# popgenmethods/smcpp

Measured on AMD Instinct MI355X. Metric: E-step loglik-evals/sec (100 Mbp, M=64, n=20), higher is better.
Workload: dtype f64 state + f32 scans (mixed)

## Files before the change

### smcpp_amd/csrc/chains_ss.hpp

```cpp
#pragma once

namespace smcpp_dev {

struct SsArgs {
    int M, Mp, nchunks, pass, K, nlds;
    const Chunk *chunks;
    const Chunk *chunks_b;
    int nchunks_b;
    const int *tasks;
    const int2 *rowdesc;
    const double *E;
    const float *pi_f;
    const double *f_dc, *f_g, *f_cg, *f_b, *f_a, *f_d;
    const double *b_dc, *b_g, *b_b, *b_a;
    double c0;
    float *alpha;
    double *beta, *cnorm;
    float *ends_f, *used_f;
    double *ends_b, *used_b;
    int *changed_f, *changed_b;
    int *endchg_f, *endchg_b;
    float eps_f;
    double eps_b;
    int full_f, full_b;
    int mode_f, mode_b;
    int halo = 0;
    long long *dbg;
    int mixed = 0;
    int dirsplit = 0;
    int hyb_th = 0x7fffffff, Ke = 0, hot_ek = 0;
    int nk_lds = 0, key_of_slot[4] = {0, 1, 2, 3}, slot_of_key[4] = {0, 1, 2, 3};
    const double *Pinvrm = nullptr, *Prm = nullptr, *PinvT = nullptr, *PT = nullptr;
    const double *dsc = nullptr;
};

constexpr int SS_KE_MAX = 4;
constexpr int SS_ROW_CONT = 1 << 30;
template <int NPL>
__device__ __forceinline__ float ss_floor_of(int descx) { return (NPL >= 2 && (descx & SS_ROW_CONT)) ? 0.f : 1e-10f; }
template <int NPL>
__device__ __forceinline__ float ss_floor_at(const SsArgs &a, long long row) { return NPL >= 2 ? ss_floor_of<NPL>(a.rowdesc[row].x) : 1e-10f; }

template <int CTRL>
__device__ __forceinline__ double dpp0(double v) {
    const long long x = __builtin_bit_cast(long long, v);
    int lo = (int)(x & 0xffffffffll), hi = (int)(x >> 32);
    lo = __builtin_amdgcn_update_dpp(0, lo, CTRL, 0xf, 0xf, true);
    hi = __builtin_amdgcn_update_dpp(0, hi, CTRL, 0xf, 0xf, true);
    return __builtin_bit_cast(double, ((long long)hi << 32) | (unsigned int)lo);
}
template <int CTRL>
__device__ __forceinline__ float dpp0(float v) {
    return __builtin_bit_cast(float, __builtin_amdgcn_update_dpp(0, __builtin_bit_cast(int, v), CTRL, 0xf, 0xf, true));
}

constexpr int DPP_SHR1 = 0x111, DPP_SHR2 = 0x112, DPP_SHR4 = 0x114, DPP_SHR8 = 0x118, DPP_BC15 = 0x142, DPP_BC31 = 0x143,
              DPP_WSHR1 = 0x138;

template <typename T>
__device__ __forceinline__ T ss_scan(T v, T c15, T c31) {
    v += dpp0<DPP_SHR1>(v);
    v += dpp0<DPP_SHR2>(v);
    v += dpp0<DPP_SHR4>(v);
    v += dpp0<DPP_SHR8>(v);
    v = __builtin_fma(c15, dpp0<DPP_BC15>(v), v);
    v = __builtin_fma(c31, dpp0<DPP_BC31>(v), v);
    return v;
}
__device__ __forceinline__ float ss_scan_f(float v, float c15, float c31) {
    v += dpp0<DPP_SHR1>(v);
    v += dpp0<DPP_SHR2>(v);
    v += dpp0<DPP_SHR4>(v);
    v += dpp0<DPP_SHR8>(v);
    v = __builtin_fmaf(c15, dpp0<DPP_BC15>(v), v);
    v = __builtin_fmaf(c31, dpp0<DPP_BC31>(v), v);
    return v;
}
__device__ __forceinline__ double ss_scan_w(double v, const double (&lv)[6]) {
    v = __builtin_fma(lv[0], dpp0<DPP_SHR1>(v), v);
    v = __builtin_fma(lv[1], dpp0<DPP_SHR2>(v), v);
    v = __builtin_fma(lv[2], dpp0<DPP_SHR4>(v), v);
    v = __builtin_fma(lv[3], dpp0<DPP_SHR8>(v), v);
    v = __builtin_fma(lv[4], dpp0<DPP_BC15>(v), v);
    v = __builtin_fma(lv[5], dpp0<DPP_BC31>(v), v);
    return v;
}
__device__ __forceinline__ void ss_levels(double A, int lane, double (&lv)[6]) {
    const int r = lane & 15, row = lane >> 4;
    double m = A, t;
    lv[0] = m; t = dpp0<DPP_SHR1>(m); m = (r >= 1) ? m * t : m;
    lv[1] = m; t = dpp0<DPP_SHR2>(m); m = (r >= 2) ? m * t : m;
    lv[2] = m; t = dpp0<DPP_SHR4>(m); m = (r >= 4) ? m * t : m;
    lv[3] = m; t = dpp0<DPP_SHR8>(m); m = (r >= 8) ? m * t : m;
    lv[4] = (row & 1) ? m : 0.0; t = dpp0<DPP_BC15>(m); m = (row & 1) ? m * t : m;
    lv[5] = (row >= 2) ? m : 0.0;
}

template <int NPL>
struct SsFwdC {
    double dc[NPL], g[NPL], cg[NPL], b[NPL], a[NPL], d[NPL], cumA[NPL], lv[6], c15, c31;
    float lvf[6];
    double adg;
    float bgf, bff, c0f, m1, m2, m3;
};
template <int NPL>
struct SsBwdC {
    double dc[NPL], g[NPL], b[NPL], a[NPL], cumA[NPL], lv[6], c15, c31, c0;
    float c15f, c31f, lvf[6];
    double adg;
    float gf, bff, c0f, m1, m2, m3;
};

template <int NPL>
__device__ __forceinline__ void ss_load_fwd(const SsArgs &a, int lane, SsFwdC<NPL> &c) {
    double cum = 1.0;
#pragma unroll
    for (int k = 0; k < NPL; ++k) {
        const int p = lane * NPL + k;
        c.dc[k] = a.f_dc[p]; c.g[k] = a.f_g[p]; c.cg[k] = a.f_cg[p]; c.b[k] = a.f_b[p]; c.a[k] = a.f_a[p]; c.d[k] = a.f_d[p];
        cum *= c.a[k];
        c.cumA[k] = cum;
    }
    ss_levels(cum, lane, c.lv);
#pragma unroll
    for (int q = 0; q < 6; ++q) c.lvf[q] = (float)c.lv[q];
    const int row = lane >> 4;
    c.c15 = (row & 1) ? 1.0 : 0.0;
    c.c31 = (row >= 2) ? 1.0 : 0.0;
    c.adg = c.d[0] - c.g[0];
    c.bgf = (float)(c.g[0] - a.c0); c.bff = (float)c.b[0]; c.c0f = (float)a.c0;
    c.m1 = row < 1 ? 1.f : 0.f; c.m2 = row < 2 ? 1.f : 0.f; c.m3 = row < 3 ? 1.f : 0.f;
}
template <int NPL>
__device__ __forceinline__ void ss_load_bwd(const SsArgs &a, int lane, SsBwdC<NPL> &c) {
    double cum = 1.0;
#pragma unroll
    for (int k = 0; k < NPL; ++k) {
        const int p = lane * NPL + k;
        c.dc[k] = a.b_dc[p]; c.g[k] = a.b_g[p]; c.b[k] = a.b_b[p]; c.a[k] = a.b_a[p];
        cum *= c.a[k];
        c.cumA[k] = cum;
    }
    ss_levels(cum, lane, c.lv);
    const int row = lane >> 4;
    c.c15 = (row & 1) ? 1.0 : 0.0;
    c.c31 = (row >= 2) ? 1.0 : 0.0;
    c.c15f = (float)c.c15; c.c31f = (float)c.c31;
#pragma unroll
    for (int q = 0; q < 6; ++q) c.lvf[q] = (float)c.lv[q];
    c.c0 = a.c0;
    c.adg = c.dc[0] - c.g[0];
    c.gf = (float)c.g[0]; c.bff = (float)c.b[0]; c.c0f = (float)a.c0;
    c.m1 = row < 1 ? 1.f : 0.f; c.m2 = row < 2 ? 1.f : 0.f; c.m3 = row < 3 ? 1.f : 0.f;
}

#define SS_D_ " row_mask:0xf bank_mask:0xf bound_ctrl:1\n"
template <bool H32>
__device__ __forceinline__ void ss_x_scan_fwd(float &z, float &s, float &zp, float &tot, const float (&lv)[6], float m1, float m2,
                                              float m3, float bg, float c0) {
    float t1, t2, t3;
    if (H32) {
        asm volatile("s_nop 1\n"
                     "v_add_f32_dpp %1, %1, %1 row_shl:1" SS_D_ "v_fmac_f32_dpp %0, %0, %5 row_shr:1" SS_D_ "s_nop 0\n"
                     "v_add_f32_dpp %1, %1, %1 row_shl:2" SS_D_ "v_fmac_f32_dpp %0, %0, %6 row_shr:2" SS_D_ "s_nop 0\n"
                     "v_add_f32_dpp %1, %1, %1 row_shl:4" SS_D_ "v_fmac_f32_dpp %0, %0, %7 row_shr:4" SS_D_ "s_nop 0\n"
                     "v_add_f32_dpp %1, %1, %1 row_shl:8" SS_D_ "v_fmac_f32_dpp %0, %0, %8 row_shr:8" SS_D_
                     "v_readlane_b32 %4, %1, 16\n"
                     "s_nop 0\n"
                     "v_fmac_f32_dpp %0, %0, %9 row_bcast:15" SS_D_
                     "v_fmac_f32_e32 %1, %4, %10\n"
                     "s_nop 0\n"
                     "v_readlane_b32 %3, %1, 0\n"
                     "v_mov_b32_dpp %2, %0 wave_shr:1" SS_D_
                     "v_fmac_f32_e32 %2, %11, %1\n"
                     "v_fmac_f32_e32 %2, %3, %12\n"
                     : "+v"(z), "+v"(s), "=&v"(zp), "=&s"(tot), "=&s"(t1)
                     : "v"(lv[0]), "v"(lv[1]), "v"(lv[2]), "v"(lv[3]), "v"(lv[4]), "v"(m1), "v"(bg), "v"(c0));
        return;
    }
    asm volatile("s_nop 1\n"
                 "v_add_f32_dpp %1, %1, %1 row_shl:1" SS_D_ "v_fmac_f32_dpp %0, %0, %7 row_shr:1" SS_D_ "s_nop 0\n"
                 "v_add_f32_dpp %1, %1, %1 row_shl:2" SS_D_ "v_fmac_f32_dpp %0, %0, %8 row_shr:2" SS_D_ "s_nop 0\n"
                 "v_add_f32_dpp %1, %1, %1 row_shl:4" SS_D_ "v_fmac_f32_dpp %0, %0, %9 row_shr:4" SS_D_ "s_nop 0\n"
                 "v_add_f32_dpp %1, %1, %1 row_shl:8" SS_D_ "v_fmac_f32_dpp %0, %0, %10 row_shr:8" SS_D_
                 "v_readlane_b32 %4, %1, 16\n"
                 "v_readlane_b32 %5, %1, 32\n"
                 "v_fmac_f32_dpp %0, %0, %11 row_bcast:15" SS_D_
                 "v_readlane_b32 %6, %1, 48\n"
                 "v_fmac_f32_e32 %1, %4, %13\n"
                 "v_fmac_f32_dpp %0, %0, %12 row_bcast:31" SS_D_
                 "v_fmac_f32_e32 %1, %5, %14\n"
                 "v_fmac_f32_e32 %1, %6, %15\n"
                 "v_mov_b32_dpp %2, %0 wave_shr:1" SS_D_
                 "v_readlane_b32 %3, %1, 0\n"
                 "v_fmac_f32_e32 %2, %16, %1\n"
                 "s_nop 0\n"
                 "v_fmac_f32_e32 %2, %3, %17\n"
                 : "+v"(z), "+v"(s), "=&v"(zp), "=&s"(tot), "=&s"(t1), "=&s"(t2), "=&s"(t3)
                 : "v"(lv[0]), "v"(lv[1]), "v"(lv[2]), "v"(lv[3]), "v"(lv[4]), "v"(lv[5]), "v"(m1), "v"(m2), "v"(m3), "v"(bg), "v"(c0));
}
template <bool H32>
__device__ __forceinline__ void ss_x_scan_bwd(float &v, float &f, float &gs, float &tot, const float (&lv)[6], float c15, float c31,
                                              float m1, float m2, float m3, float b, float c0) {
    float t1, t2, t3, vp;
    if (H32) {
        asm volatile("s_nop 1\n"
                     "v_add_f32_dpp %1, %0, %0 row_shr:1" SS_D_ "v_add_f32_dpp %2, %2, %2 row_shl:1" SS_D_ "v_fmac_f32_dpp %0, %0, %6 row_shr:1" SS_D_
                     "v_add_f32_dpp %1, %1, %1 row_shr:2" SS_D_ "v_add_f32_dpp %2, %2, %2 row_shl:2" SS_D_ "v_fmac_f32_dpp %0, %0, %7 row_shr:2" SS_D_
                     "v_add_f32_dpp %1, %1, %1 row_shr:4" SS_D_ "v_add_f32_dpp %2, %2, %2 row_shl:4" SS_D_ "v_fmac_f32_dpp %0, %0, %8 row_shr:4" SS_D_
                     "v_add_f32_dpp %1, %1, %1 row_shr:8" SS_D_ "v_add_f32_dpp %2, %2, %2 row_shl:8" SS_D_ "v_fmac_f32_dpp %0, %0, %9 row_shr:8" SS_D_
                     "v_readlane_b32 %5, %2, 48\n"
                     "v_fmac_f32_dpp %1, %1, %11 row_bcast:15" SS_D_
                     "v_fmac_f32_dpp %0, %0, %10 row_bcast:15" SS_D_
                     "v_fmac_f32_e32 %2, %5, %12\n"
                     "v_readlane_b32 %3, %1, 63\n"
                     "v_mov_b32_dpp %4, %0 wave_shr:1" SS_D_
                     "v_fmac_f32_e32 %2, %14, %1\n"
                     "v_fmac_f32_e32 %2, %13, %4\n"
                     : "+v"(v), "=&v"(f), "+v"(gs), "=&s"(tot), "=&v"(vp), "=&s"(t3)
                     : "v"(lv[0]), "v"(lv[1]), "v"(lv[2]), "v"(lv[3]), "v"(lv[4]), "v"(c15), "v"(m3), "v"(b), "v"(c0));
        return;
    }
    asm volatile("s_nop 1\n"
                 "v_add_f32_dpp %1, %0, %0 row_shr:1" SS_D_ "v_add_f32_dpp %2, %2, %2 row_shl:1" SS_D_ "v_fmac_f32_dpp %0, %0, %8 row_shr:1" SS_D_
                 "v_add_f32_dpp %1, %1, %1 row_shr:2" SS_D_ "v_add_f32_dpp %2, %2, %2 row_shl:2" SS_D_ "v_fmac_f32_dpp %0, %0, %9 row_shr:2" SS_D_
                 "v_add_f32_dpp %1, %1, %1 row_shr:4" SS_D_ "v_add_f32_dpp %2, %2, %2 row_shl:4" SS_D_ "v_fmac_f32_dpp %0, %0, %10 row_shr:4" SS_D_
                 "v_add_f32_dpp %1, %1, %1 row_shr:8" SS_D_ "v_add_f32_dpp %2, %2, %2 row_shl:8" SS_D_ "v_fmac_f32_dpp %0, %0, %11 row_shr:8" SS_D_
                 "v_readlane_b32 %5, %2, 16\n"
                 "v_fmac_f32_dpp %1, %1, %14 row_bcast:15" SS_D_
                 "v_fmac_f32_dpp %0, %0, %12 row_bcast:15" SS_D_
                 "v_readlane_b32 %6, %2, 32\n"
                 "v_readlane_b32 %7, %2, 48\n"
                 "v_fmac_f32_dpp %1, %1, %15 row_bcast:31" SS_D_
                 "v_fmac_f32_dpp %0, %0, %13 row_bcast:31" SS_D_
                 "v_fmac_f32_e32 %2, %5, %16\n"
                 "v_fmac_f32_e32 %2, %6, %17\n"
                 "v_fmac_f32_e32 %2, %7, %18\n"
                 "v_mov_b32_dpp %4, %0 wave_shr:1" SS_D_
                 "v_readlane_b32 %3, %1, 63\n"
                 "v_fmac_f32_e32 %2, %20, %1\n"
                 "v_fmac_f32_e32 %2, %19, %4\n"
                 : "+v"(v), "=&v"(f), "+v"(gs), "=&s"(tot), "=&v"(vp), "=&s"(t1), "=&s"(t2), "=&s"(t3)
                 : "v"(lv[0]), "v"(lv[1]), "v"(lv[2]), "v"(lv[3]), "v"(lv[4]), "v"(lv[5]), "v"(c15), "v"(c31), "v"(m1), "v"(m2), "v"(m3),
                   "v"(b), "v"(c0));
}
#undef SS_D_

template <int NPL, bool MIX = false, bool H32 = false>
__device__ __forceinline__ void ss_fwd_step(const SsFwdC<NPL> &c, const double (&x)[NPL], const double (&e)[NPL],
                                            double (&out)[NPL], double &S) {
    if (MIX && NPL == 1) {
        float s = (float)x[0];
        float z = c.bff * s, zp, tot;
        ss_x_scan_fwd<H32>(z, s, zp, tot, c.lvf, c.m1, c.m2, c.m3, c.bgf, c.c0f);
        S = (double)tot;
        out[0] = e[0] * __builtin_fma(c.adg, x[0], (double)zp);
        return;
    }
    double lp[NPL], w[NPL];
    lp[0] = x[0];
    w[0] = c.b[0] * x[0];
#pragma unroll
    for (int k = 1; k < NPL; ++k) {
        lp[k] = lp[k - 1] + x[k];
        w[k] = __builtin_fma(c.a[k], w[k - 1], c.b[k] * x[k]);
    }
    double p_ = lp[NPL - 1], z_ = w[NPL - 1];
    {
        double tp, tz;
        tp = dpp0<DPP_SHR1>(p_); tz = dpp0<DPP_SHR1>(z_); p_ += tp; z_ = __builtin_fma(c.lv[0], tz, z_);
        tp = dpp0<DPP_SHR2>(p_); tz = dpp0<DPP_SHR2>(z_); p_ += tp; z_ = __builtin_fma(c.lv[1], tz, z_);
        tp = dpp0<DPP_SHR4>(p_); tz = dpp0<DPP_SHR4>(z_); p_ += tp; z_ = __builtin_fma(c.lv[2], tz, z_);
        tp = dpp0<DPP_SHR8>(p_); tz = dpp0<DPP_SHR8>(z_); p_ += tp; z_ = __builtin_fma(c.lv[3], tz, z_);
        tp = dpp0<DPP_BC15>(p_); tz = dpp0<DPP_BC15>(z_); p_ = __builtin_fma(c.c15, tp, p_); z_ = __builtin_fma(c.lv[4], tz, z_);
        tp = dpp0<DPP_BC31>(p_); tz = dpp0<DPP_BC31>(z_); p_ = __builtin_fma(c.c31, tp, p_); z_ = __builtin_fma(c.lv[5], tz, z_);
    }
    const double li = p_, LI = z_;
    S = lane_get(li, 63);
    const double LIp = dpp0<DPP_WSHR1>(LI);
    if (NPL == 1) {
        out[0] = e[0] * __builtin_fma(c.dc[0], x[0], __builtin_fma(c.g[0], S, __builtin_fma(c.cg[0], li, LIp)));
        return;
    }
    const double lex = li - lp[NPL - 1];
#pragma unroll
    for (int k = 0; k < NPL; ++k) {
        const double incl = lex + lp[k];
        const double Z = (k == 0) ? LIp : __builtin_fma(c.cumA[k - 1 < 0 ? 0 : k - 1], LIp, w[k - 1 < 0 ? 0 : k - 1]);
        const double t = __builtin_fma(c.dc[k], x[k], __builtin_fma(c.g[k], S, __builtin_fma(c.cg[k], incl, Z)));
        out[k] = e[k] * t;
    }
}

template <int NPL, bool MIX = false, bool H32 = false>
__device__ __forceinline__ void ss_bwd_step(const SsBwdC<NPL> &c, const double (&bv)[NPL], const double (&e)[NPL],
                                            double (&out)[NPL], float &Sw) {
    if (MIX && NPL == 1) {
        const double w0 = e[0] * bv[0];
        float v = (float)w0;
        float gs = c.gf * v, f;
        ss_x_scan_bwd<H32>(v, f, gs, Sw, c.lvf, c.c15f, c.c31f, c.m1, c.m2, c.m3, c.bff, c.c0f);
        out[0] = __builtin_fma(c.adg, w0, (double)gs);
        return;
    }
    double w[NPL], lg[NPL], u[NPL];
    float lf[NPL];
#pragma unroll
    for (int k = 0; k < NPL; ++k) w[k] = e[k] * bv[k];
    lg[0] = c.g[0] * w[0];
    u[0] = w[0];
    lf[0] = (float)w[0];
#pragma unroll
    for (int k = 1; k < NPL; ++k) {
        lg[k] = __builtin_fma(c.g[k], w[k], lg[k - 1]);
        u[k] = __builtin_fma(c.a[k], u[k - 1], w[k]);
        lf[k] = lf[k - 1] + (float)w[k];
    }
    double p_ = lg[NPL - 1], z_ = u[NPL - 1];
    float f_ = lf[NPL - 1];
    {
        double tp, tz;
        float tf;
        tp = dpp0<DPP_SHR1>(p_); tz = dpp0<DPP_SHR1>(z_); tf = dpp0<DPP_SHR1>(f_); p_ += tp; z_ = __builtin_fma(c.lv[0], tz, z_); f_ += tf;
        tp = dpp0<DPP_SHR2>(p_); tz = dpp0<DPP_SHR2>(z_); tf = dpp0<DPP_SHR2>(f_); p_ += tp; z_ = __builtin_fma(c.lv[1], tz, z_); f_ += tf;
        tp = dpp0<DPP_SHR4>(p_); tz = dpp0<DPP_SHR4>(z_); tf = dpp0<DPP_SHR4>(f_); p_ += tp; z_ = __builtin_fma(c.lv[2], tz, z_); f_ += tf;
        tp = dpp0<DPP_SHR8>(p_); tz = dpp0<DPP_SHR8>(z_); tf = dpp0<DPP_SHR8>(f_); p_ += tp; z_ = __builtin_fma(c.lv[3], tz, z_); f_ += tf;
        tp = dpp0<DPP_BC15>(p_); tz = dpp0<DPP_BC15>(z_); tf = dpp0<DPP_BC15>(f_);
        p_ = __builtin_fma(c.c15, tp, p_); z_ = __builtin_fma(c.lv[4], tz, z_); f_ = __builtin_fmaf(c.c15f, tf, f_);
        tp = dpp0<DPP_BC31>(p_); tz = dpp0<DPP_BC31>(z_); tf = dpp0<DPP_BC31>(f_);
        p_ = __builtin_fma(c.c31, tp, p_); z_ = __builtin_fma(c.lv[5], tz, z_); f_ = __builtin_fmaf(c.c31f, tf, f_);
    }
    const double lig = p_, LI = z_;
    const float lif = f_;
    const double Gtot = lane_get(lig, 63);
    Sw = lane_get(lif, 63);
    const double LIp = dpp0<DPP_WSHR1>(LI);
    if (NPL == 1) {
        out[0] = __builtin_fma(c.dc[0], w[0], (Gtot - lig) + __builtin_fma(c.c0, (double)lif, c.b[0] * LIp));
        return;
    }
    const double lexg = lig - lg[NPL - 1];
    const float lexf = lif - lf[NPL - 1];
#pragma unroll
    for (int k = 0; k < NPL; ++k) {
        const double inclG = lexg + lg[k];
        const double inclW = (double)(lexf + lf[k]);
        const double V = (k == 0) ? LIp : __builtin_fma(c.cumA[k - 1 < 0 ? 0 : k - 1], LIp, u[k - 1 < 0 ? 0 : k - 1]);
        out[k] = __builtin_fma(c.dc[k], w[k], (Gtot - inclG) + __builtin_fma(c.c0, inclW, c.b[k] * V));
    }
}

__device__ __forceinline__ void ss_desc_settle(int2 &d) { asm volatile("" : "+v"(d.x), "+v"(d.y)); }
__device__ __forceinline__ void ss_vm_drain() { __builtin_amdgcn_s_waitcnt(0x0F70); }
__device__ __forceinline__ int ss_uni(int v) { return __builtin_amdgcn_readfirstlane(v); }
__device__ __forceinline__ Chunk ss_uniform_chunk(const Chunk &c) {
    Chunk u;
    const unsigned lo = (unsigned)__builtin_amdgcn_readfirstlane((int)(c.base & 0xffffffffll));
    const unsigned hi = (unsigned)__builtin_amdgcn_readfirstlane((int)(c.base >> 32));
    u.base = (long long)(((unsigned long long)hi << 32) | lo);
    u.r0 = ss_uni(c.r0); u.r1 = ss_uni(c.r1); u.contig = ss_uni(c.contig); u.first = ss_uni(c.first); u.last = ss_uni(c.last);
    u.pad = ss_uni(c.pad); u.h0 = ss_uni(c.h0); u.h1 = ss_uni(c.h1);
    return u;
}

template <int NPL, bool BWD, bool ALLLDS = false>
__device__ __forceinline__ void ss_emission(const SsArgs &a, const double *sE, int slot, int lane, double (&e)[NPL]) {
    constexpr int MS = 64 * NPL;
    if (ALLLDS || slot < a.nlds) {
        const double *src = sE + (size_t)slot * MS;
#pragma unroll
        for (int k = 0; k < NPL; ++k) e[k] = src[BWD ? MS - 1 - (lane * NPL + k) : lane * NPL + k];
    } else {
        const double *src = a.E + (size_t)slot * MS;
#pragma unroll
        for (int k = 0; k < NPL; ++k) e[k] = src[BWD ? MS - 1 - (lane * NPL + k) : lane * NPL + k];
    }
}

__device__ __forceinline__ double ss_sum_halves(double v) {
    const long long x = __builtin_bit_cast(long long, v);
    const int lo = (int)(x & 0xffffffffll), hi = (int)(x >> 32);
    const auto r0 = __builtin_amdgcn_permlane32_swap(lo, lo, false, false);
    const auto r1 = __builtin_amdgcn_permlane32_swap(hi, hi, false, false);
    const double a = __builtin_bit_cast(double, ((long long)(unsigned)r1[0] << 32) | (unsigned)r0[0]);
    const double b = __builtin_bit_cast(double, ((long long)(unsigned)r1[1] << 32) | (unsigned)r0[1]);
    return a + b;
}
__device__ __forceinline__ double ss_exp_neg(double x) {
    if (!(x > -745.0)) return 0.0;
    const double n = __builtin_rint(x * 1.4426950408889634);
    double r = __builtin_fma(-n, 6.93147180369123816490e-01, x);
    r = __builtin_fma(-n, 1.90821492927058770002e-10, r);
    double p = 1.0 / 6227020800.0;
    p = __builtin_fma(p, r, 1.0 / 479001600.0);
    p = __builtin_fma(p, r, 1.0 / 39916800.0);
    p = __builtin_fma(p, r, 1.0 / 3628800.0);
    p = __builtin_fma(p, r, 1.0 / 362880.0);
    p = __builtin_fma(p, r, 1.0 / 40320.0);
    p = __builtin_fma(p, r, 1.0 / 5040.0);
    p = __builtin_fma(p, r, 1.0 / 720.0);
    p = __builtin_fma(p, r, 1.0 / 120.0);
    p = __builtin_fma(p, r, 1.0 / 24.0);
    p = __builtin_fma(p, r, 1.0 / 6.0);
    p = __builtin_fma(p, r, 0.5);
    p = __builtin_fma(p, r, 1.0);
    p = __builtin_fma(p, r, 1.0);
    return ldexp(p, (int)n);
}
struct SsEigC { double ld[SS_KE_MAX]; bool neg[SS_KE_MAX]; int slot[SS_KE_MAX]; int r, g, nb, G, tpk; };
__device__ __forceinline__ void ss_load_eig(const SsArgs &a, int lp, SsEigC &c) {
    c.G = a.Mp <= 32 ? 2 : 1;
    c.tpk = a.dirsplit ? 2 : 4;
    const int W = 64 / c.G;
    c.r = lp & (W - 1); c.g = lp / W; c.nb = a.Mp / c.G;
#pragma unroll
    for (int e = 0; e < SS_KE_MAX; ++e) {
        double d = 0.0;
        if (e < a.Ke && c.r < a.M) d = a.dsc[(size_t)e * a.Mp + c.r];
        c.ld[e] = log(fabs(d));
        c.neg[e] = d < 0.0;
        c.slot[e] = a.slot_of_key[e];
    }
}
__device__ __forceinline__ double ss_eig_pow(const SsEigC &c, int ek, int span) {
    double l = c.ld[0];
    bool ng = c.neg[0];
#pragma unroll
    for (int e = 1; e < SS_KE_MAX; ++e) if (ek == e) { l = c.ld[e]; ng = c.neg[e]; }
    const double p = ss_exp_neg((double)span * l);
    return (ng && (span & 1)) ? -p : p;
}
__device__ __forceinline__ double ss_eig_matvec(const SsEigC &c, const double *tab, int Mp, int slot, int which, double *sx, int lp, double x) {
    sx[lp] = x;
    wave_lds_fence();
    const double *row = tab + ((size_t)(slot * c.tpk + (which & (c.tpk - 1))) * Mp + min(c.r, Mp - 1)) * (Mp + 1) + c.g * c.nb;
    const double *xv = sx + c.g * c.nb;
    double a0 = 0.0, a1 = 0.0;
    for (int b = 0; b < c.nb; b += 4) {
        const double r0 = row[b], r1 = row[b + 1], r2 = row[b + 2], r3 = row[b + 3];
        const double v0 = xv[b], v1 = xv[b + 1], v2 = xv[b + 2], v3 = xv[b + 3];
        a0 = __builtin_fma(r0, v0, a0); a1 = __builtin_fma(r1, v1, a1);
        a0 = __builtin_fma(r2, v2, a0); a1 = __builtin_fma(r3, v3, a1);
    }
    double acc = a0 + a1;
    if (c.G >= 2) acc = ss_sum_halves(acc);
    wave_lds_fence();
    return acc;
}
__device__ __forceinline__ double ss_eig_matvec_cold(const SsEigC &c, const double *mat, int Mp, double *sx, int lp, double x) {
    sx[lp] = x;
    wave_lds_fence();
    const double *row = mat + (size_t)min(c.r, Mp - 1) * Mp + c.g * c.nb;
    const double *xv = sx + c.g * c.nb;
    double a0 = 0.0, a1 = 0.0;
    for (int b = 0; b < c.nb; b += 8) {
        double rr[8];
#pragma unroll
        for (int q = 0; q < 8; ++q) rr[q] = row[b + q];
#pragma unroll
        for (int q = 0; q < 8; q += 2) { a0 = __builtin_fma(rr[q], xv[b + q], a0); a1 = __builtin_fma(rr[q + 1], xv[b + q + 1], a1); }
    }
    double acc = a0 + a1;
    if (c.G >= 2) acc = ss_sum_halves(acc);
    wave_lds_fence();
    return acc;
}

template <int NB>
struct SsHotRows { double a[NB], b[NB]; };
template <int NB>
__device__ __forceinline__ void ss_eig_rows(const SsEigC &c, const double *tab, int Mp, int ek, int w0, double (&ra)[NB], double (&rb)[NB]) {
    const size_t rowoff = (size_t)min(c.r, Mp - 1) * (Mp + 1) + c.g * NB;
    const double *rowA = tab + (size_t)(ek * c.tpk + (w0 & (c.tpk - 1))) * Mp * (Mp + 1) + rowoff;
    const double *rowB = tab + (size_t)(ek * c.tpk + (w0 & (c.tpk - 1)) + 1) * Mp * (Mp + 1) + rowoff;
#pragma unroll
    for (int b = 0; b < NB; ++b) { ra[b] = rowA[b]; rb[b] = rowB[b]; }
}
template <int NB>
__device__ __forceinline__ double ss_eig_step(const SsEigC &c, const double *tab, int Mp, int ek, int w0, double *sx, int lp,
                                              double xin, int span, const SsHotRows<NB> &hot, int hot_ek) {
    double ra[NB], rb[NB];
    if (ek == hot_ek) {
#pragma unroll
        for (int b = 0; b < NB; ++b) { ra[b] = hot.a[b]; rb[b] = hot.b[b]; }
    } else ss_eig_rows<NB>(c, tab, Mp, ek, w0, ra, rb);
    sx[lp] = xin;
    const double pw = ss_eig_pow(c, ek, span);
    wave_lds_fence();
    const double *xv = sx + c.g * NB;
    double a0 = 0.0, a1 = 0.0;
#pragma unroll
    for (int b = 0; b < NB; b += 2) { a0 = __builtin_fma(ra[b], xv[b], a0); a1 = __builtin_fma(ra[b + 1], xv[b + 1], a1); }
    const double u = ss_sum_halves(a0 + a1) * pw;
    wave_lds_fence();
    sx[c.r] = u;
    wave_lds_fence();
    a0 = 0.0; a1 = 0.0;
#pragma unroll
    for (int b = 0; b < NB; b += 2) { a0 = __builtin_fma(rb[b], xv[b], a0); a1 = __builtin_fma(rb[b + 1], xv[b + 1], a1); }
    const double o = ss_sum_halves(a0 + a1);
    wave_lds_fence();
    return o;
}
__device__ __forceinline__ double ss_eig_apply(const SsArgs &a, const SsEigC &c, const double *tab, int Mp, int ek, int w0, double *sx, int lp,
                                               double xin, int span, const SsHotRows<16> &hot, int hot_ek) {
    if (Mp == 32) return ss_eig_step<16>(c, tab, Mp, ek, w0, sx, lp, xin, span, hot, hot_ek);
    if (Mp == 16) {
        SsHotRows<8> none;
        return ss_eig_step<8>(c, tab, Mp, ek, w0, sx, lp, xin, span, none, -1);
    }
    int slot = c.slot[0];
#pragma unroll
    for (int e = 1; e < SS_KE_MAX; ++e) if (ek == e) slot = c.slot[e];
    if (slot >= 0) {
        double u = ss_eig_matvec(c, tab, Mp, slot, w0, sx, lp, xin);
        u *= ss_eig_pow(c, ek, span);
        return ss_eig_matvec(c, tab, Mp, slot, w0 + 1, sx, lp, lp < 64 / c.G ? u : 0.0);
    }
    const size_t MM = (size_t)Mp * Mp;
    const double *m0 = (w0 == 0 ? a.Pinvrm : a.PT) + (size_t)ek * MM, *m1 = (w0 == 0 ? a.Prm : a.PinvT) + (size_t)ek * MM;
    double u = ss_eig_matvec_cold(c, m0, Mp, sx, lp, xin);
    u *= ss_eig_pow(c, ek, span);
    return ss_eig_matvec_cold(c, m1, Mp, sx, lp, lp < 64 / c.G ? u : 0.0);
}

template <int NPL, bool ALLLDS>
__device__ __forceinline__ void ss_fwd_light_rows(const SsArgs &a, const double *sE, long long base, int first, int last, int lane, float (&x)[NPL]);
template <int NPL, bool ALLLDS>
__device__ __forceinline__ void ss_bwd_light_rows(const SsArgs &a, const double *sE, long long base, int rhi, int rlo, int lane, float (&b)[NPL]);

template <int NPL, bool RERUN, bool HYB, bool ALLLDS, bool MIX = false, bool H32 = false>
__device__ __forceinline__ void ss_forward_wave(const SsArgs &a, const double *sE, int c, int lane) {
    constexpr int MS = 64 * NPL;
    const int M = a.M, Mp = a.Mp, pass = a.pass;
    const Chunk ch = ss_uniform_chunk(a.chunks[c]);
    float *end_cur = a.ends_f + ((size_t)(pass & 1) * a.nchunks + c) * Mp;
    const float *end_prev = a.ends_f + ((size_t)((pass + 1) & 1) * a.nchunks + c) * Mp;
    int st[NPL];
    bool live[NPL], stor[NPL];
#pragma unroll
    for (int k = 0; k < NPL; ++k) { st[k] = lane * NPL + k; live[k] = st[k] < M; stor[k] = st[k] < Mp; }
    if (RERUN && ch.first && !a.full_f) {
#pragma unroll
        for (int k = 0; k < NPL; ++k) if (stor[k]) end_cur[st[k]] = end_prev[st[k]];
        return;
    }
    double x[NPL];
    {
        const float *src = (ch.first || !RERUN) ? a.pi_f : a.ends_f + ((size_t)((pass + 1) & 1) * a.nchunks + (c - 1)) * Mp;
#pragma unroll
        for (int k = 0; k < NPL; ++k) x[k] = live[k] ? (double)src[st[k]] : 0.0;
    }
    const bool halo = !RERUN && !HYB && a.halo && ch.h0 < ch.r0;
    const int rbeg = halo ? ch.h1 : ch.r0;
    const int jst = ch.r0 - rbeg;
    if (halo && ch.h0 < ch.h1) {
        float xf[NPL];
#pragma unroll
        for (int k = 0; k < NPL; ++k) xf[k] = (float)x[k];
        ss_fwd_light_rows<NPL, ALLLDS>(a, sE, ch.base, ch.h0, ch.h1, lane, xf);
#pragma unroll
        for (int k = 0; k < NPL; ++k) x[k] = live[k] ? (double)xf[k] : 0.0;
        if (jst == 0) {
            double part = 0.0;
#pragma unroll
            for (int k = 0; k < NPL; ++k) part += x[k];
            const double iv = 1.0 / wave_sum_dpp(part);
#pragma unroll
            for (int k = 0; k < NPL; ++k) {
                const float an = live[k] ? fmaxf((float)(x[k] * iv), ss_floor_at<NPL>(a, ch.base + ch.r0 + 1)) : 0.f;
                x[k] = (double)an;
                if (stor[k]) a.used_f[(size_t)c * Mp + st[k]] = an;
            }
        }
    }
    if (RERUN && !a.full_f) {
        bool diff = false;
#pragma unroll
        for (int k = 0; k < NPL; ++k)
            if (live[k]) {
                const float u = a.used_f[(size_t)c * Mp + st[k]];
                if (!(fabsf((float)x[k] - u) <= a.eps_f * fabsf(u))) diff = true;
            }
        if (!__any(diff)) {
#pragma unroll
            for (int k = 0; k < NPL; ++k) if (stor[k]) end_cur[st[k]] = end_prev[st[k]];
            return;
        }
    }
    if (!halo) {
#pragma unroll
        for (int k = 0; k < NPL; ++k) if (stor[k]) a.used_f[(size_t)c * Mp + st[k]] = (float)x[k];
    }
    if (lane == 0) a.changed_f[pass] = 1;
    if (ch.first) {
#pragma unroll
        for (int k = 0; k < NPL; ++k) if (stor[k]) a.alpha[(size_t)ch.base * Mp + st[k]] = (float)x[k];
        if (lane == 0) a.cnorm[ch.base] = 1.0;
    }
    SsFwdC<NPL> cst;
    ss_load_fwd<NPL>(a, lane, cst);
    const int2 *rd = a.rowdesc + ch.base + rbeg + 1;
    const int nrows = ch.r1 - rbeg;
    int2 dcur = rd[lane], dnxt = rd[64 + lane];
    ss_desc_settle(dcur); ss_desc_settle(dnxt);
    float *arow = a.alpha + (size_t)(ch.base + rbeg) * Mp;
    double *crow = a.cnorm + ch.base + rbeg;
    float *ap[NPL];
#pragma unroll
    for (int k = 0; k < NPL; ++k) ap[k] = arow + st[k];
    int cacc = 0;
    auto cflush = [&](int jhi) {
        const int jj = (jhi & ~63) + lane;
        if (jj <= jhi && jj > jst && jj > 0) crow[jj] = (double)__builtin_bit_cast(float, cacc);
    };
    double e[NPL];
    ss_emission<NPL, false, ALLLDS>(a, sE, __builtin_amdgcn_readlane(dcur.x, 0) & 0xFFFF, lane, e);
    constexpr bool hyb = HYB && NPL == 1;
    const double *tab = sE + (size_t)a.nlds * MS;
    SsEigC ec;
    SsHotRows<16> hot;
    int hot_ek = -1;
    if (hyb) {
        ss_load_eig(a, lane, ec);
        if (Mp == 32) { hot_ek = a.hot_ek; ss_eig_rows<16>(ec, tab, Mp, hot_ek, 0, hot.a, hot.b); }
    }
    double *sxw = const_cast<double *>(tab) + (size_t)a.nk_lds * (a.dirsplit ? 2 : 4) * Mp * (Mp + 1) + (threadIdx.x >> 6) * 64;
    bool merged = false;
    const long long t0c = __builtin_readcyclecounter(), t0r = __builtin_amdgcn_s_memrealtime();
    long long npos = 0;
    ss_vm_drain();
    for (int j = 0; j < nrows; ++j) {
        const int jl = j & 63;
        const int span = __builtin_amdgcn_readlane(dcur.y, jl);
        const int ekr = (__builtin_amdgcn_readlane(dcur.x, jl) >> 16) & 0xFF;
        const float flo = NPL >= 2 ? ss_floor_of<NPL>(__builtin_amdgcn_readlane(dcur.x, jl)) : 1e-10f;
        npos += span;
        if (jl == 63) { dcur = dnxt; dnxt = rd[j + 65 + lane]; ss_desc_settle(dnxt); }
        if (MIX && jl == 0 && j > 0) cflush(j - 1);
        const int slot_n = __builtin_amdgcn_readlane(dcur.x, (j + 1) & 63) & 0xFFFF;
        double en[NPL];
        ss_emission<NPL, false, ALLLDS>(a, sE, slot_n, lane, en);
        if (hyb && span > a.hyb_th) {
            const double S = wave_sum_dpp(x[0]);
            const double inv = rcp_f64(S);
            double xin = x[0] * inv;
            if (j > 0) {
                const float an = live[0] ? fmaxf((float)xin, flo) : 0.f;
                if (RERUN && !a.full_f && (j & 15) == 0 && j >= 16) {
                    bool bad = false;
                    if (live[0]) {
                        const float old = arow[(size_t)j * Mp + st[0]];
                        if (!(fabsf(an - old) <= a.eps_f * fabsf(old))) bad = true;
                    }
                    if (!__any(bad)) { merged = true; break; }
                }
                if (stor[0]) arow[(size_t)j * Mp + st[0]] = an;
                if (lane == 0) crow[j] = S;
                xin = (double)an;
            }
            const double xo = ss_eig_apply(a, ec, tab, Mp, ekr, 0, sxw, lane, xin, span, hot, hot_ek);
            x[0] = live[0] ? xo : 0.0;
#pragma unroll
            for (int k = 0; k < NPL; ++k) e[k] = en[k];
            continue;
        }
        double y[NPL], S;
        ss_fwd_step<NPL, MIX, MIX && H32>(cst, x, e, y, S);
        double inv;
        if (MIX) {
            const double r0 = (double)__builtin_amdgcn_rcpf((float)S);
            inv = __builtin_fma(__builtin_fma(-S, r0, 1.0), r0, r0);
        } else inv = rcp_f64(S);
        double fb[NPL];
#pragma unroll
        for (int k = 0; k < NPL; ++k) fb[k] = 0.0;
        if (j > 0) {
            float an[NPL];
#pragma unroll
            for (int k = 0; k < NPL; ++k) {
                const double xs = x[k] * inv;
                an[k] = live[k] ? fmaxf((float)xs, flo) : 0.f;
                fb[k] = (double)an[k] - xs;
            }
            if (RERUN && !a.full_f && (j & 15) == 0 && j >= 16) {
                bool bad = false;
#pragma unroll
                for (int k = 0; k < NPL; ++k)
                    if (live[k]) {
                        const float old = MIX ? *ap[k] : arow[(size_t)j * Mp + st[k]];
                        if (!(fabsf(an[k] - old) <= a.eps_f * fabsf(old))) bad = true;
                    }
                if (!__any(bad)) { merged = true; if (MIX) cflush(j - 1); break; }
            }
            if (j > jst) {
                if (MIX) {
#pragma unroll
                    for (int k = 0; k < NPL; ++k) if (stor[k]) *ap[k] = an[k];
                    cacc = lane == jl ? __builtin_bit_cast(int, (float)S) : cacc;
                } else {
#pragma unroll
                    for (int k = 0; k < NPL; ++k) if (stor[k]) arow[(size_t)j * Mp + st[k]] = an[k];
                    if (lane == 0) crow[j] = S;
                }
            } else if (j == jst) {
#pragma unroll
                for (int k = 0; k < NPL; ++k) if (stor[k]) a.used_f[(size_t)c * Mp + st[k]] = an[k];
            }
        }
#pragma unroll
        for (int k = 0; k < NPL; ++k) {
            double ed = e[k] * cst.d[k];
            if (span == 1) { const double edf = (double)(float)ed; y[k] = __builtin_fma(edf - ed, x[k], y[k]); ed = edf; }
            x[k] = __builtin_fma(ed, fb[k], y[k] * inv);
        }
        {
            double S2;
            int t = 1;
            for (; t + 1 < span; t += 2) {
                ss_fwd_step<NPL, MIX, MIX && H32>(cst, x, e, y, S2);
#pragma unroll
                for (int k = 0; k < NPL; ++k) x[k] = y[k];
                ss_fwd_step<NPL, MIX, MIX && H32>(cst, x, e, y, S2);
#pragma unroll
                for (int k = 0; k < NPL; ++k) x[k] = y[k];
            }
            if (t < span) {
                ss_fwd_step<NPL, MIX, MIX && H32>(cst, x, e, y, S2);
#pragma unroll
                for (int k = 0; k < NPL; ++k) x[k] = y[k];
            }
        }
#pragma unroll
        for (int k = 0; k < NPL; ++k) e[k] = en[k];
        if (MIX) {
#pragma unroll
            for (int k = 0; k < NPL; ++k) ap[k] += Mp;
        }
    }
    if (MIX && !merged && nrows > 0) cflush(nrows - 1);
    if (a.dbg && !RERUN && c == 1 && lane == 0) {
        a.dbg[0] = __builtin_readcyclecounter() - t0c; a.dbg[1] = __builtin_amdgcn_s_memrealtime() - t0r;
        a.dbg[2] = npos; a.dbg[3] = nrows;
    }
    if (merged) {
#pragma unroll
        for (int k = 0; k < NPL; ++k) if (stor[k]) end_cur[st[k]] = end_prev[st[k]];
        return;
    }
    {
        double part = 0.0;
#pragma unroll
        for (int k = 0; k < NPL; ++k) part += x[k];
        const double S = wave_sum_dpp(part);
        const double inv = 1.0 / S;
#pragma unroll
        for (int k = 0; k < NPL; ++k) {
            const float an = live[k] ? fmaxf((float)(x[k] * inv), ss_floor_at<NPL>(a, ch.base + ch.r1 + 1)) : 0.f;
            if (stor[k]) { a.alpha[(size_t)(ch.base + ch.r1) * Mp + st[k]] = an; end_cur[st[k]] = an; }
        }
        if (lane == 0) { a.cnorm[ch.base + ch.r1] = S; a.endchg_f[pass] = 1; }
    }
}

template <int NPL, bool RERUN, bool HYB, bool ALLLDS, bool MIX = false, bool H32 = false>
__device__ __forceinline__ void ss_backward_wave(const SsArgs &a, const double *sE, int c, int lane) {
    constexpr int MS = 64 * NPL;
    const int M = a.M, Mp = a.Mp, pass = a.pass;
    const Chunk ch = ss_uniform_chunk(a.chunks_b[c]);
    double *end_cur = a.ends_b + ((size_t)(pass & 1) * a.nchunks_b + c) * Mp;
    const double *end_prev = a.ends_b + ((size_t)((pass + 1) & 1) * a.nchunks_b + c) * Mp;
    int st[NPL];
    bool live[NPL], stor[NPL];
#pragma unroll
    for (int k = 0; k < NPL; ++k) { st[k] = MS - 1 - (lane * NPL + k); live[k] = st[k] < M; stor[k] = st[k] < Mp; }
    if (RERUN && ch.last && !a.full_b) {
#pragma unroll
        for (int k = 0; k < NPL; ++k) if (stor[k]) end_cur[st[k]] = end_prev[st[k]];
        return;
    }
    double b[NPL];
    {
        const bool fresh = ch.last || !RERUN;
        const double *src = a.ends_b + ((size_t)((pass + 1) & 1) * a.nchunks_b + (fresh ? c : c + 1)) * Mp;
#pragma unroll
        for (int k = 0; k < NPL; ++k) b[k] = live[k] ? (fresh ? 1.0 / (double)M : src[st[k]]) : 0.0;
    }
    const bool halo = !RERUN && !HYB && a.halo && ch.h0 > ch.r1;
    const int rend = halo ? ch.h1 : ch.r1;
    const int jst = rend - ch.r1;
    if (halo && ch.h0 > ch.h1) {
        float bf_[NPL];
#pragma unroll
        for (int k = 0; k < NPL; ++k) bf_[k] = (float)b[k];
        ss_bwd_light_rows<NPL, ALLLDS>(a, sE, ch.base, ch.h0, ch.h1, lane, bf_);
        float pt = 0.f;
#pragma unroll
        for (int k = 0; k < NPL; ++k) pt += live[k] ? bf_[k] : 0.f;
        const float iv = 1.f / wave_sum_dpp(pt);
#pragma unroll
        for (int k = 0; k < NPL; ++k) b[k] = live[k] ? (double)(bf_[k] * iv) : 0.0;
    }
    if (RERUN && !a.full_b) {
        bool diff = false;
#pragma unroll
        for (int k = 0; k < NPL; ++k)
            if (live[k]) {
                const double u = a.used_b[(size_t)c * Mp + st[k]];
                if (!(fabs(b[k] - u) <= a.eps_b * fabs(u))) diff = true;
            }
        if (!__any(diff)) {
#pragma unroll
            for (int k = 0; k < NPL; ++k) if (stor[k]) end_cur[st[k]] = end_prev[st[k]];
            return;
        }
    }
    if (!halo) {
#pragma unroll
        for (int k = 0; k < NPL; ++k) if (stor[k]) a.used_b[(size_t)c * Mp + st[k]] = b[k];
    }
    if (lane == 0) a.changed_b[pass] = 1;
    SsBwdC<NPL> cst;
    ss_load_bwd<NPL>(a, lane, cst);
    const int2 *rd = a.rowdesc + ch.base + rend;
    const int nrows = rend - ch.r0;
    int2 dcur = rd[-lane], dnxt = rd[-64 - lane];
    ss_desc_settle(dcur); ss_desc_settle(dnxt);
    double *brow = a.beta + (size_t)(ch.base + rend) * Mp;
    double *bp[NPL];
#pragma unroll
    for (int k = 0; k < NPL; ++k) bp[k] = brow + st[k];
    double e[NPL];
    ss_emission<NPL, true, ALLLDS>(a, sE, __builtin_amdgcn_readlane(dcur.x, 0) & 0xFFFF, lane, e);
    constexpr bool hyb = HYB && NPL == 1;
    const double *tab = sE + (size_t)a.nlds * MS;
    SsEigC ec;
    SsHotRows<16> hot;
    int hot_ek = -1;
    if (hyb) {
        ss_load_eig(a, 63 - lane, ec);
        if (Mp == 32) { hot_ek = a.hot_ek; ss_eig_rows<16>(ec, tab, Mp, hot_ek, 2, hot.a, hot.b); }
    }
    double *sxw = const_cast<double *>(tab) + (size_t)a.nk_lds * (a.dirsplit ? 2 : 4) * Mp * (Mp + 1) + (threadIdx.x >> 6) * 64;
    bool merged = false;
    const long long t0c = __builtin_readcyclecounter(), t0r = __builtin_amdgcn_s_memrealtime();
    long long npos = 0;
    ss_vm_drain();
    for (int j = 0; j < nrows; ++j) {
        const int jl = j & 63;
        const int span = __builtin_amdgcn_readlane(dcur.y, jl);
        const int ekr = (__builtin_amdgcn_readlane(dcur.x, jl) >> 16) & 0xFF;
        npos += span;
        if (jl == 63) { dcur = dnxt; dnxt = rd[-(j + 65) - lane]; ss_desc_settle(dnxt); }
        const int slot_n = __builtin_amdgcn_readlane(dcur.x, (j + 1) & 63) & 0xFFFF;
        double en[NPL];
        ss_emission<NPL, true, ALLLDS>(a, sE, slot_n, lane, en);
        if (RERUN && !a.full_b && (j & 15) == 0 && j >= 16) {
            bool bad = false;
#pragma unroll
            for (int k = 0; k < NPL; ++k)
                if (live[k]) {
                    const double old = MIX ? *bp[k] : brow[-(ptrdiff_t)j * Mp + st[k]];
                    if (!(fabs(b[k] - old) <= a.eps_b * fabs(old))) bad = true;
                }
            if (!__any(bad)) { merged = true; break; }
        }
        if (halo && j == jst) {
            double part = 0.0;
#pragma unroll
            for (int k = 0; k < NPL; ++k) part += live[k] ? b[k] : 0.0;
            const double iv = 1.0 / wave_sum_dpp(part);
#pragma unroll
            for (int k = 0; k < NPL; ++k) {
                b[k] = live[k] ? b[k] * iv : 0.0;
                if (stor[k]) a.used_b[(size_t)c * Mp + st[k]] = b[k];
            }
        }
        if (j >= jst) {
#pragma unroll
            for (int k = 0; k < NPL; ++k) if (stor[k]) { if (MIX) *bp[k] = b[k]; else brow[-(ptrdiff_t)j * Mp + st[k]] = b[k]; }
        }
        if (hyb && span > a.hyb_th) {
            const double bin = live[0] ? b[0] : 0.0;
            double bo = ss_eig_apply(a, ec, tab, Mp, ekr, 2, sxw, 63 - lane, bin, span, hot, hot_ek);
            bo = live[0] ? bo : 0.0;
            b[0] = bo * rcp_f64(wave_sum_dpp(bo));
#pragma unroll
            for (int k = 0; k < NPL; ++k) e[k] = en[k];
            continue;
        }
        double y[NPL];
        float Sw;
        ss_bwd_step<NPL, MIX, MIX && H32>(cst, b, e, y, Sw);
        const double inv = (double)__builtin_amdgcn_rcpf(Sw);
#pragma unroll
        for (int k = 0; k < NPL; ++k) b[k] = y[k] * inv;
        {
            float S2;
            int t = 1;
            for (; t + 1 < span; t += 2) {
                ss_bwd_step<NPL, MIX, MIX && H32>(cst, b, e, y, S2);
#pragma unroll
                for (int k = 0; k < NPL; ++k) b[k] = y[k];
                ss_bwd_step<NPL, MIX, MIX && H32>(cst, b, e, y, S2);
#pragma unroll
                for (int k = 0; k < NPL; ++k) b[k] = y[k];
            }
            if (t < span) {
                ss_bwd_step<NPL, MIX, MIX && H32>(cst, b, e, y, S2);
#pragma unroll
                for (int k = 0; k < NPL; ++k) b[k] = y[k];
            }
        }
#pragma unroll
        for (int k = 0; k < NPL; ++k) e[k] = en[k];
        if (MIX) {
#pragma unroll
            for (int k = 0; k < NPL; ++k) bp[k] -= Mp;
        }
    }
    if (a.dbg && !RERUN && c == 1 && lane == 0) {
        a.dbg[4] = __builtin_readcyclecounter() - t0c; a.dbg[5] = __builtin_amdgcn_s_memrealtime() - t0r;
        a.dbg[6] = npos; a.dbg[7] = nrows;
    }
    if (merged) {
#pragma unroll
        for (int k = 0; k < NPL; ++k) if (stor[k]) end_cur[st[k]] = end_prev[st[k]];
        return;
    }
    {
        double part = 0.0;
#pragma unroll
        for (int k = 0; k < NPL; ++k) part += live[k] ? b[k] : 0.0;
        const double S = wave_sum_dpp(part);
#pragma unroll
        for (int k = 0; k < NPL; ++k) {
            const double bf = live[k] ? b[k] / S : 0.0;
            if (stor[k]) { end_cur[st[k]] = bf; if (ch.first) a.beta[(size_t)ch.base * Mp + st[k]] = bf; }
        }
        if (lane == 0) a.endchg_b[pass] = 1;
    }
}

template <int NPL>
struct SsLightC { float dc[NPL], g[NPL], cg[NPL], b[NPL], a[NPL], cumA[NPL], lv[6], c15, c31, c0; };

template <int NPL, bool BWD>
__device__ __forceinline__ void ss_load_light(const SsArgs &a, int lane, SsLightC<NPL> &c) {
    double cum = 1.0;
#pragma unroll
    for (int k = 0; k < NPL; ++k) {
        const int p = lane * NPL + k;
        c.dc[k] = (float)(BWD ? a.b_dc[p] : a.f_dc[p]);
        c.g[k] = (float)(BWD ? a.b_g[p] : a.f_g[p]);
        c.cg[k] = BWD ? 0.f : (float)a.f_cg[p];
        c.b[k] = (float)(BWD ? a.b_b[p] : a.f_b[p]);
        const double av = BWD ? a.b_a[p] : a.f_a[p];
        c.a[k] = (float)av;
        cum *= av;
        c.cumA[k] = (float)cum;
    }
    double lv[6];
    ss_levels(cum, lane, lv);
#pragma unroll
    for (int q = 0; q < 6; ++q) c.lv[q] = (float)lv[q];
    const int row = lane >> 4;
    c.c15 = (row & 1) ? 1.f : 0.f;
    c.c31 = (row >= 2) ? 1.f : 0.f;
    c.c0 = (float)a.c0;
}

#define SS_DPP_ "row_mask:0xf bank_mask:0xf bound_ctrl:1\n"
template <bool H32>
__device__ __forceinline__ void ss_light_scan2(float &p, float &z, const float (&lv)[6], float c15, float c31) {
    if (H32) {
        asm volatile("s_nop 1\n"
                     "v_add_f32_dpp %0, %0, %0 row_shr:1 " SS_DPP_ "v_fmac_f32_dpp %1, %1, %2 row_shr:1 " SS_DPP_ "s_nop 0\n"
                     "v_add_f32_dpp %0, %0, %0 row_shr:2 " SS_DPP_ "v_fmac_f32_dpp %1, %1, %3 row_shr:2 " SS_DPP_ "s_nop 0\n"
                     "v_add_f32_dpp %0, %0, %0 row_shr:4 " SS_DPP_ "v_fmac_f32_dpp %1, %1, %4 row_shr:4 " SS_DPP_ "s_nop 0\n"
                     "v_add_f32_dpp %0, %0, %0 row_shr:8 " SS_DPP_ "v_fmac_f32_dpp %1, %1, %5 row_shr:8 " SS_DPP_ "s_nop 0\n"
                     "v_fmac_f32_dpp %0, %0, %7 row_bcast:15 " SS_DPP_ "v_fmac_f32_dpp %1, %1, %6 row_bcast:15 " SS_DPP_ "s_nop 1\n"
                     : "+v"(p), "+v"(z)
                     : "v"(lv[0]), "v"(lv[1]), "v"(lv[2]), "v"(lv[3]), "v"(lv[4]), "v"(c15));
        return;
    }
    asm volatile("s_nop 1\n"
                 "v_add_f32_dpp %0, %0, %0 row_shr:1 " SS_DPP_ "v_fmac_f32_dpp %1, %1, %2 row_shr:1 " SS_DPP_ "s_nop 0\n"
                 "v_add_f32_dpp %0, %0, %0 row_shr:2 " SS_DPP_ "v_fmac_f32_dpp %1, %1, %3 row_shr:2 " SS_DPP_ "s_nop 0\n"
                 "v_add_f32_dpp %0, %0, %0 row_shr:4 " SS_DPP_ "v_fmac_f32_dpp %1, %1, %4 row_shr:4 " SS_DPP_ "s_nop 0\n"
                 "v_add_f32_dpp %0, %0, %0 row_shr:8 " SS_DPP_ "v_fmac_f32_dpp %1, %1, %5 row_shr:8 " SS_DPP_ "s_nop 0\n"
                 "v_fmac_f32_dpp %0, %0, %8 row_bcast:15 " SS_DPP_ "v_fmac_f32_dpp %1, %1, %6 row_bcast:15 " SS_DPP_ "s_nop 0\n"
                 "v_fmac_f32_dpp %0, %0, %9 row_bcast:31 " SS_DPP_ "v_fmac_f32_dpp %1, %1, %7 row_bcast:31 " SS_DPP_ "s_nop 1\n"
                 : "+v"(p), "+v"(z)
                 : "v"(lv[0]), "v"(lv[1]), "v"(lv[2]), "v"(lv[3]), "v"(lv[4]), "v"(lv[5]), "v"(c15), "v"(c31));
}
template <bool H32>
__device__ __forceinline__ void ss_light_scan3(float &p, float &z, float &f, const float (&lv)[6], float c15, float c31) {
    if (H32) {
        asm volatile("s_nop 1\n"
                     "v_add_f32_dpp %0, %0, %0 row_shr:1 " SS_DPP_ "v_fmac_f32_dpp %1, %1, %3 row_shr:1 " SS_DPP_ "v_add_f32_dpp %2, %2, %2 row_shr:1 " SS_DPP_
                     "v_add_f32_dpp %0, %0, %0 row_shr:2 " SS_DPP_ "v_fmac_f32_dpp %1, %1, %4 row_shr:2 " SS_DPP_ "v_add_f32_dpp %2, %2, %2 row_shr:2 " SS_DPP_
                     "v_add_f32_dpp %0, %0, %0 row_shr:4 " SS_DPP_ "v_fmac_f32_dpp %1, %1, %5 row_shr:4 " SS_DPP_ "v_add_f32_dpp %2, %2, %2 row_shr:4 " SS_DPP_
                     "v_add_f32_dpp %0, %0, %0 row_shr:8 " SS_DPP_ "v_fmac_f32_dpp %1, %1, %6 row_shr:8 " SS_DPP_ "v_add_f32_dpp %2, %2, %2 row_shr:8 " SS_DPP_
                     "v_fmac_f32_dpp %0, %0, %8 row_bcast:15 " SS_DPP_ "v_fmac_f32_dpp %1, %1, %7 row_bcast:15 " SS_DPP_ "v_fmac_f32_dpp %2, %2, %8 row_bcast:15 " SS_DPP_ "s_nop 1\n"
                     : "+v"(p), "+v"(z), "+v"(f)
                     : "v"(lv[0]), "v"(lv[1]), "v"(lv[2]), "v"(lv[3]), "v"(lv[4]), "v"(c15));
        return;
    }
    asm volatile("s_nop 1\n"
                 "v_add_f32_dpp %0, %0, %0 row_shr:1 " SS_DPP_ "v_fmac_f32_dpp %1, %1, %3 row_shr:1 " SS_DPP_ "v_add_f32_dpp %2, %2, %2 row_shr:1 " SS_DPP_
                 "v_add_f32_dpp %0, %0, %0 row_shr:2 " SS_DPP_ "v_fmac_f32_dpp %1, %1, %4 row_shr:2 " SS_DPP_ "v_add_f32_dpp %2, %2, %2 row_shr:2 " SS_DPP_
                 "v_add_f32_dpp %0, %0, %0 row_shr:4 " SS_DPP_ "v_fmac_f32_dpp %1, %1, %5 row_shr:4 " SS_DPP_ "v_add_f32_dpp %2, %2, %2 row_shr:4 " SS_DPP_
                 "v_add_f32_dpp %0, %0, %0 row_shr:8 " SS_DPP_ "v_fmac_f32_dpp %1, %1, %6 row_shr:8 " SS_DPP_ "v_add_f32_dpp %2, %2, %2 row_shr:8 " SS_DPP_
                 "v_fmac_f32_dpp %0, %0, %9 row_bcast:15 " SS_DPP_ "v_fmac_f32_dpp %1, %1, %7 row_bcast:15 " SS_DPP_ "v_fmac_f32_dpp %2, %2, %9 row_bcast:15 " SS_DPP_
                 "v_fmac_f32_dpp %0, %0, %10 row_bcast:31 " SS_DPP_ "v_fmac_f32_dpp %1, %1, %8 row_bcast:31 " SS_DPP_ "v_fmac_f32_dpp %2, %2, %10 row_bcast:31 " SS_DPP_ "s_nop 1\n"
                 : "+v"(p), "+v"(z), "+v"(f)
                 : "v"(lv[0]), "v"(lv[1]), "v"(lv[2]), "v"(lv[3]), "v"(lv[4]), "v"(lv[5]), "v"(c15), "v"(c31));
}
#undef SS_DPP_

template <int NPL, bool H32 = false>
__device__ __forceinline__ void ss_fwd_step_f(const SsLightC<NPL> &c, const float (&x)[NPL], const float (&e)[NPL],
                                              float (&out)[NPL], float &S) {
    float lp[NPL], w[NPL];
    lp[0] = x[0];
    w[0] = c.b[0] * x[0];
#pragma unroll
    for (int k = 1; k < NPL; ++k) {
        lp[k] = lp[k - 1] + x[k];
        w[k] = __builtin_fmaf(c.a[k], w[k - 1], c.b[k] * x[k]);
    }
    float p_ = lp[NPL - 1], z_ = w[NPL - 1];
    ss_light_scan2<H32>(p_, z_, c.lv, c.c15, c.c31);
    S = lane_get(p_, H32 ? 31 : 63);
    const float LIp = dpp0<DPP_WSHR1>(z_);
    if (NPL == 1) {
        out[0] = e[0] * __builtin_fmaf(c.dc[0], x[0], __builtin_fmaf(c.g[0], S, __builtin_fmaf(c.cg[0], p_, LIp)));
        return;
    }
    const float lex = p_ - lp[NPL - 1];
#pragma unroll
    for (int k = 0; k < NPL; ++k) {
        const float incl = lex + lp[k];
        const float Z = (k == 0) ? LIp : __builtin_fmaf(c.cumA[k - 1 < 0 ? 0 : k - 1], LIp, w[k - 1 < 0 ? 0 : k - 1]);
        out[k] = e[k] * __builtin_fmaf(c.dc[k], x[k], __builtin_fmaf(c.g[k], S, __builtin_fmaf(c.cg[k], incl, Z)));
    }
}

template <int NPL, bool H32 = false>
__device__ __forceinline__ void ss_bwd_step_f(const SsLightC<NPL> &c, const float (&bv)[NPL], const float (&e)[NPL],
                                              float (&out)[NPL], float &Sw) {
    float w[NPL], lg[NPL], u[NPL], lf[NPL];
#pragma unroll
    for (int k = 0; k < NPL; ++k) w[k] = e[k] * bv[k];
    lg[0] = c.g[0] * w[0];
    u[0] = w[0];
    lf[0] = w[0];
#pragma unroll
    for (int k = 1; k < NPL; ++k) {
        lg[k] = __builtin_fmaf(c.g[k], w[k], lg[k - 1]);
        u[k] = __builtin_fmaf(c.a[k], u[k - 1], w[k]);
        lf[k] = lf[k - 1] + w[k];
    }
    float p_ = lg[NPL - 1], z_ = u[NPL - 1], f_ = lf[NPL - 1];
    ss_light_scan3<H32>(p_, z_, f_, c.lv, c.c15, c.c31);
    const float Gtot = lane_get(p_, 63);
    Sw = lane_get(f_, 63);
    const float LIp = dpp0<DPP_WSHR1>(z_);
    if (NPL == 1) {
        out[0] = __builtin_fmaf(c.dc[0], w[0], (Gtot - p_) + __builtin_fmaf(c.c0, f_, c.b[0] * LIp));
        return;
    }
    const float lexg = p_ - lg[NPL - 1], lexf = f_ - lf[NPL - 1];
#pragma unroll
    for (int k = 0; k < NPL; ++k) {
        const float inclG = lexg + lg[k], inclW = lexf + lf[k];
        const float V = (k == 0) ? LIp : __builtin_fmaf(c.cumA[k - 1 < 0 ? 0 : k - 1], LIp, u[k - 1 < 0 ? 0 : k - 1]);
        out[k] = __builtin_fmaf(c.dc[k], w[k], (Gtot - inclG) + __builtin_fmaf(c.c0, inclW, c.b[k] * V));
    }
}

template <int NPL, bool BWD, bool ALLLDS>
__device__ __forceinline__ void ss_emission_f(const SsArgs &a, const double *sE, int slot, int lane, float (&e)[NPL]) {
    double ed[NPL];
    ss_emission<NPL, BWD, ALLLDS>(a, sE, slot, lane, ed);
#pragma unroll
    for (int k = 0; k < NPL; ++k) e[k] = (float)ed[k];
}

template <int NPL, bool ALLLDS>
__device__ __forceinline__ void ss_fwd_light_rows(const SsArgs &a, const double *sE, long long base, int first, int last, int lane,
                                                  float (&x)[NPL]) {
    SsLightC<NPL> cst;
    ss_load_light<NPL, false>(a, lane, cst);
    const int2 *rd = a.rowdesc + base + first + 1;
    const int nrows = last - first;
    int2 dcur = rd[lane], dnxt = rd[64 + lane];
    ss_desc_settle(dcur); ss_desc_settle(dnxt);
    float e[NPL];
    ss_emission_f<NPL, false, ALLLDS>(a, sE, __builtin_amdgcn_readlane(dcur.x, 0) & 0xFFFF, lane, e);
    ss_vm_drain();
    for (int j = 0; j < nrows; ++j) {
        const int jl = j & 63;
        const int span = __builtin_amdgcn_readlane(dcur.y, jl);
        if (jl == 63) { dcur = dnxt; dnxt = rd[j + 65 + lane]; ss_desc_settle(dnxt); }
        const int slot_n = __builtin_amdgcn_readlane(dcur.x, (j + 1) & 63) & 0xFFFF;
        float en[NPL], y[NPL], S;
        ss_emission_f<NPL, false, ALLLDS>(a, sE, slot_n, lane, en);
        ss_fwd_step_f<NPL>(cst, x, e, y, S);
        const float inv = __builtin_amdgcn_rcpf(S);
#pragma unroll
        for (int k = 0; k < NPL; ++k) x[k] = y[k] * inv;
        float S2;
        int t = 1;
        for (; t + 1 < span; t += 2) {
            ss_fwd_step_f<NPL>(cst, x, e, y, S2);
#pragma unroll
            for (int k = 0; k < NPL; ++k) x[k] = y[k];
            ss_fwd_step_f<NPL>(cst, x, e, y, S2);
#pragma unroll
            for (int k = 0; k < NPL; ++k) x[k] = y[k];
        }
        if (t < span) {
            ss_fwd_step_f<NPL>(cst, x, e, y, S2);
#pragma unroll
            for (int k = 0; k < NPL; ++k) x[k] = y[k];
        }
#pragma unroll
        for (int k = 0; k < NPL; ++k) e[k] = en[k];
    }
}
template <int NPL, bool ALLLDS>
__device__ __forceinline__ void ss_bwd_light_rows(const SsArgs &a, const double *sE, long long base, int rhi, int rlo, int lane,
                                                  float (&b)[NPL]) {
    SsLightC<NPL> cst;
    ss_load_light<NPL, true>(a, lane, cst);
    const int2 *rd = a.rowdesc + base + rhi;
    const int nrows = rhi - rlo;
    int2 dcur = rd[-lane], dnxt = rd[-64 - lane];
    ss_desc_settle(dcur); ss_desc_settle(dnxt);
    float e[NPL];
    ss_emission_f<NPL, true, ALLLDS>(a, sE, __builtin_amdgcn_readlane(dcur.x, 0) & 0xFFFF, lane, e);
    ss_vm_drain();
    for (int j = 0; j < nrows; ++j) {
        const int jl = j & 63;
        const int span = __builtin_amdgcn_readlane(dcur.y, jl);
        if (jl == 63) { dcur = dnxt; dnxt = rd[-(j + 65) - lane]; ss_desc_settle(dnxt); }
        const int slot_n = __builtin_amdgcn_readlane(dcur.x, (j + 1) & 63) & 0xFFFF;
        float en[NPL], y[NPL], Sw;
        ss_emission_f<NPL, true, ALLLDS>(a, sE, slot_n, lane, en);
        ss_bwd_step_f<NPL>(cst, b, e, y, Sw);
        const float inv = __builtin_amdgcn_rcpf(Sw);
#pragma unroll
        for (int k = 0; k < NPL; ++k) b[k] = y[k] * inv;
        float S2;
        int t = 1;
        for (; t + 1 < span; t += 2) {
            ss_bwd_step_f<NPL>(cst, b, e, y, S2);
#pragma unroll
            for (int k = 0; k < NPL; ++k) b[k] = y[k];
            ss_bwd_step_f<NPL>(cst, b, e, y, S2);
#pragma unroll
            for (int k = 0; k < NPL; ++k) b[k] = y[k];
        }
        if (t < span) {
            ss_bwd_step_f<NPL>(cst, b, e, y, S2);
#pragma unroll
            for (int k = 0; k < NPL; ++k) b[k] = y[k];
        }
#pragma unroll
        for (int k = 0; k < NPL; ++k) e[k] = en[k];
    }
}

template <int NPL, bool ALLLDS, bool H32 = false>
__device__ __forceinline__ void ss_forward_light(const SsArgs &a, const double *sE, int c, int lane) {
    const int M = a.M, Mp = a.Mp, pass = a.pass;
    const Chunk ch = ss_uniform_chunk(a.chunks[c]);
    float *end_cur = a.ends_f + ((size_t)(pass & 1) * a.nchunks + c) * Mp;
    int st[NPL];
    bool live[NPL], stor[NPL];
#pragma unroll
    for (int k = 0; k < NPL; ++k) { st[k] = lane * NPL + k; live[k] = st[k] < M; stor[k] = st[k] < Mp; }
    float x[NPL];
    {
        const float *src = (ch.first || pass == 0) ? a.pi_f : a.ends_f + ((size_t)((pass + 1) & 1) * a.nchunks + (c - 1)) * Mp;
#pragma unroll
        for (int k = 0; k < NPL; ++k) x[k] = live[k] ? src[st[k]] : 0.f;
    }
    if (lane == 0) { a.changed_f[pass] = 1; a.endchg_f[pass] = 1; }
    SsLightC<NPL> cst;
    ss_load_light<NPL, false>(a, lane, cst);
    const int2 *rd = a.rowdesc + ch.base + ch.r0 + 1;
    const int nrows = ch.r1 - ch.r0;
    int2 dcur = rd[lane], dnxt = rd[64 + lane];
    ss_desc_settle(dcur); ss_desc_settle(dnxt);
    float e[NPL];
    ss_emission_f<NPL, false, ALLLDS>(a, sE, __builtin_amdgcn_readlane(dcur.x, 0) & 0xFFFF, lane, e);
    ss_vm_drain();
    for (int j = 0; j < nrows; ++j) {
        const int jl = j & 63;
        const int span = __builtin_amdgcn_readlane(dcur.y, jl);
        if (jl == 63) { dcur = dnxt; dnxt = rd[j + 65 + lane]; ss_desc_settle(dnxt); }
        const int slot_n = __builtin_amdgcn_readlane(dcur.x, (j + 1) & 63) & 0xFFFF;
        float en[NPL], y[NPL], S;
        ss_emission_f<NPL, false, ALLLDS>(a, sE, slot_n, lane, en);
        ss_fwd_step_f<NPL, H32>(cst, x, e, y, S);
        const float inv = __builtin_amdgcn_rcpf(S);
#pragma unroll
        for (int k = 0; k < NPL; ++k) x[k] = y[k] * inv;
        {
            float S2;
            int t = 1;
            for (; t + 1 < span; t += 2) {
                ss_fwd_step_f<NPL, H32>(cst, x, e, y, S2);
#pragma unroll
                for (int k = 0; k < NPL; ++k) x[k] = y[k];
                ss_fwd_step_f<NPL, H32>(cst, x, e, y, S2);
#pragma unroll
                for (int k = 0; k < NPL; ++k) x[k] = y[k];
            }
            if (t < span) {
                ss_fwd_step_f<NPL, H32>(cst, x, e, y, S2);
#pragma unroll
                for (int k = 0; k < NPL; ++k) x[k] = y[k];
            }
        }
#pragma unroll
        for (int k = 0; k < NPL; ++k) e[k] = en[k];
    }
    float part = 0.f;
#pragma unroll
    for (int k = 0; k < NPL; ++k) part += x[k];
    const float inv = 1.f / wave_sum_dpp(part);
#pragma unroll
    for (int k = 0; k < NPL; ++k) if (stor[k]) end_cur[st[k]] = live[k] ? fmaxf(x[k] * inv, ss_floor_at<NPL>(a, ch.base + ch.r1 + 1)) : 0.f;
}

template <int NPL, bool ALLLDS, bool H32 = false>
__device__ __forceinline__ void ss_backward_light(const SsArgs &a, const double *sE, int c, int lane) {
    constexpr int MS = 64 * NPL;
    const int M = a.M, Mp = a.Mp, pass = a.pass;
    const Chunk ch = ss_uniform_chunk(a.chunks_b[c]);
    double *end_cur = a.ends_b + ((size_t)(pass & 1) * a.nchunks_b + c) * Mp;
    int st[NPL];
    bool live[NPL], stor[NPL];
#pragma unroll
    for (int k = 0; k < NPL; ++k) { st[k] = MS - 1 - (lane * NPL + k); live[k] = st[k] < M; stor[k] = st[k] < Mp; }
    float b[NPL];
    {
        const bool fresh = ch.last || pass == 0;
        const double *src = a.ends_b + ((size_t)((pass + 1) & 1) * a.nchunks_b + (fresh ? c : c + 1)) * Mp;
#pragma unroll
        for (int k = 0; k < NPL; ++k) b[k] = live[k] ? (fresh ? 1.f / (float)M : (float)src[st[k]]) : 0.f;
    }
    if (lane == 0) { a.changed_b[pass] = 1; a.endchg_b[pass] = 1; }
    SsLightC<NPL> cst;
    ss_load_light<NPL, true>(a, lane, cst);
    const int2 *rd = a.rowdesc + ch.base + ch.r1;
    const int nrows = ch.r1 - ch.r0;
    int2 dcur = rd[-lane], dnxt = rd[-64 - lane];
    ss_desc_settle(dcur); ss_desc_settle(dnxt);
    float e[NPL];
    ss_emission_f<NPL, true, ALLLDS>(a, sE, __builtin_amdgcn_readlane(dcur.x, 0) & 0xFFFF, lane, e);
    ss_vm_drain();
    for (int j = 0; j < nrows; ++j) {
        const int jl = j & 63;
        const int span = __builtin_amdgcn_readlane(dcur.y, jl);
        if (jl == 63) { dcur = dnxt; dnxt = rd[-(j + 65) - lane]; ss_desc_settle(dnxt); }
        const int slot_n = __builtin_amdgcn_readlane(dcur.x, (j + 1) & 63) & 0xFFFF;
        float en[NPL], y[NPL], Sw;
        ss_emission_f<NPL, true, ALLLDS>(a, sE, slot_n, lane, en);
        ss_bwd_step_f<NPL, H32>(cst, b, e, y, Sw);
        const float inv = __builtin_amdgcn_rcpf(Sw);
#pragma unroll
        for (int k = 0; k < NPL; ++k) b[k] = y[k] * inv;
        {
            float S2;
            int t = 1;
            for (; t + 1 < span; t += 2) {
                ss_bwd_step_f<NPL, H32>(cst, b, e, y, S2);
#pragma unroll
                for (int k = 0; k < NPL; ++k) b[k] = y[k];
                ss_bwd_step_f<NPL, H32>(cst, b, e, y, S2);
#pragma unroll
                for (int k = 0; k < NPL; ++k) b[k] = y[k];
            }
            if (t < span) {
                ss_bwd_step_f<NPL, H32>(cst, b, e, y, S2);
#pragma unroll
                for (int k = 0; k < NPL; ++k) b[k] = y[k];
            }
        }
#pragma unroll
        for (int k = 0; k < NPL; ++k) e[k] = en[k];
    }
    float part = 0.f;
#pragma unroll
    for (int k = 0; k < NPL; ++k) part += live[k] ? b[k] : 0.f;
    const float inv = 1.f / wave_sum_dpp(part);
#pragma unroll
    for (int k = 0; k < NPL; ++k) if (stor[k]) end_cur[st[k]] = live[k] ? (double)(b[k] * inv) : 0.0;
}

template <int NPL, bool HYB, bool ALLLDS, bool H32 = false>
__global__ __launch_bounds__(HYB ? 512 : 256) void k_chain_ss(SsArgs a) {
    constexpr int MS = 64 * NPL;
    extern __shared__ __attribute__((aligned(16))) double ss_lds[];
    const int tid = threadIdx.x, lane = tid & 63, w = tid >> 6;
    const bool idle_f = (a.mode_f == 1 && !a.full_f && a.changed_f[a.pass - 1] == 0);
    const bool idle_b = (a.mode_b == 1 && !a.full_b && a.changed_b[a.pass - 1] == 0);
    if (idle_f && idle_b) return;
    const int nthr = HYB ? (int)blockDim.x : 256;
    for (int idx = tid; idx < a.nlds * MS; idx += nthr) ss_lds[idx] = a.E[idx];
    if (HYB && NPL == 1) {
        double *tab = ss_lds + (size_t)a.nlds * MS;
        const int Mp = a.Mp, MM = Mp * Mp;
        if (a.dirsplit) {
            const int nw = nthr >> 6;
            int t0 = -1;
            for (int i = 0; i < nw && t0 < 0; ++i) t0 = a.tasks[nw * blockIdx.x + i];
            const bool wg_bwd = t0 >= 0 && (t0 >> 30);
            for (int idx = tid; idx < a.nk_lds * 2 * MM; idx += nthr) {
                const int mat = idx / MM, rc = idx % MM, r = rc / Mp, cc = rc % Mp;
                const int e = a.key_of_slot[mat >> 1], which = (mat & 1) + (wg_bwd ? 2 : 0);
                const double *src = which == 0 ? a.Pinvrm : which == 1 ? a.Prm : which == 2 ? a.PT : a.PinvT;
                tab[((size_t)mat * Mp + r) * (Mp + 1) + cc] = src[(size_t)e * MM + rc];
            }
        } else
        for (int idx = tid; idx < a.nk_lds * 4 * MM; idx += nthr) {
            const int mat = idx / MM, rc = idx % MM, r = rc / Mp, cc = rc % Mp;
            const int e = a.key_of_slot[mat >> 2], which = mat & 3;
            const double *src = which == 0 ? a.Pinvrm : which == 1 ? a.Prm : which == 2 ? a.PT : a.PinvT;
            tab[((size_t)mat * Mp + r) * (Mp + 1) + cc] = src[(size_t)e * MM + rc];
        }
    }
    __syncthreads();
    const int task = ss_uni(a.tasks[(nthr >> 6) * blockIdx.x + w]);
    if (task < 0) return;
    const bool fwd = !(task >> 30);
    const int c = task & 0x3FFFFFFF;
    if (fwd) {
        if (idle_f) return;
        if (NPL == 1 && !HYB && a.mixed) {
            if (a.mode_f == 0) ss_forward_wave<NPL, false, HYB, ALLLDS, true, H32>(a, ss_lds, c, lane);
            else if (a.mode_f == 1) ss_forward_wave<NPL, true, HYB, ALLLDS, true, H32>(a, ss_lds, c, lane);
            else ss_forward_light<NPL, ALLLDS, H32>(a, ss_lds, c, lane);
        } else
        if (a.mode_f == 0) ss_forward_wave<NPL, false, HYB, ALLLDS>(a, ss_lds, c, lane);
        else if (a.mode_f == 1) ss_forward_wave<NPL, true, HYB, ALLLDS>(a, ss_lds, c, lane);
        else ss_forward_light<NPL, ALLLDS, H32>(a, ss_lds, c, lane);
    } else {
        if (idle_b) return;
        if (NPL == 1 && !HYB && a.mixed) {
            if (a.mode_b == 0) ss_backward_wave<NPL, false, HYB, ALLLDS, true, H32>(a, ss_lds, c, lane);
            else if (a.mode_b == 1) ss_backward_wave<NPL, true, HYB, ALLLDS, true, H32>(a, ss_lds, c, lane);
            else ss_backward_light<NPL, ALLLDS, H32>(a, ss_lds, c, lane);
        } else
        if (a.mode_b == 0) ss_backward_wave<NPL, false, HYB, ALLLDS>(a, ss_lds, c, lane);
        else if (a.mode_b == 1) ss_backward_wave<NPL, true, HYB, ALLLDS>(a, ss_lds, c, lane);
        else ss_backward_light<NPL, ALLLDS, H32>(a, ss_lds, c, lane);
    }
}

template <int NPL, int PHASE>
__global__ __launch_bounds__(256) void k_span_scan(SsArgs sa, FinArgs a, int smax, double *__restrict__ Fall) {
    constexpr int MS = 64 * NPL;
    const int lane = threadIdx.x & 63;
    const int gw = blockIdx.x * 4 + (threadIdx.x >> 6);
    const int M = a.M, Mp = a.Mp;
    const int ce = ss_uni(gw / M), rc = ss_uni(gw % M);
    if (ce >= a.n_contigs * a.Ke) return;
    const int b0 = ss_uni(a.ce_bucket_off[ce]), b1 = ss_uni(a.ce_bucket_off[ce + 1]);
    if (b0 == b1) return;
    const int e = ce % a.Ke;
    const double *ek = a.E + (size_t)a.e_kid[e] * Mp;
    double *Fce = Fall + (size_t)ce * smax * Mp * Mp;
    int st[NPL];
    bool live[NPL];
    double ev[NPL];
#pragma unroll
    for (int k = 0; k < NPL; ++k) {
        const int p = lane * NPL + k;
        st[k] = PHASE == 0 ? MS - 1 - p : p;
        live[k] = st[k] < M;
        ev[k] = live[k] ? ek[st[k]] : 0.0;
    }
    double x[NPL];
#pragma unroll
    for (int k = 0; k < NPL; ++k) x[k] = 0.0;
    if (PHASE == 0) {
        int mybk = -1;
        for (int b = b0; b < b1; ++b) {
            const int sp = a.g_span[a.eb_gid[b]];
            if (sp - 1 == lane) mybk = b;
        }
        SsBwdC<NPL> c;
        ss_load_bwd<NPL>(sa, lane, c);
        auto fetch = [&](int t, double (&v)[NPL]) {
            const int bk = __builtin_amdgcn_readlane(mybk, max(t, 0));
            const double *src = a.red_e + (size_t)max(bk, b0) * Mp * Mp + (size_t)rc * Mp;
#pragma unroll
            for (int k = 0; k < NPL; ++k) v[k] = src[min(st[k], Mp - 1)];
            return bk;
        };
        double nx[NPL];
        int bkn = fetch(smax - 1, nx);
        for (int t = smax - 1; t >= 0; --t) {
            double cur[NPL], out[NPL];
            const bool has = bkn >= 0;
#pragma unroll
            for (int k = 0; k < NPL; ++k) cur[k] = (has && live[k]) ? nx[k] : 0.0;
            bkn = fetch(t - 1, nx);
            float Sw;
            ss_bwd_step<NPL>(c, x, ev, out, Sw);
            double *Ft = Fce + (size_t)t * Mp * Mp;
#pragma unroll
            for (int k = 0; k < NPL; ++k) {
                x[k] = out[k] + cur[k];
                if (live[k]) Ft[(size_t)st[k] * Mp + rc] = x[k];
            }
        }
        return;
    }
    SsFwdC<NPL> c;
    ss_load_fwd<NPL>(sa, lane, c);
    auto fetchF = [&](int t, double (&v)[NPL]) {
        const double *src = Fce + (size_t)max(t, 0) * Mp * Mp + (size_t)rc * Mp;
#pragma unroll
        for (int k = 0; k < NPL; ++k) v[k] = src[min(st[k], Mp - 1)];
    };
    double nx[NPL];
    fetchF(smax - 1, nx);
    for (int t = smax - 1; t >= 0; --t) {
        double cur[NPL], out[NPL], S;
#pragma unroll
        for (int k = 0; k < NPL; ++k) cur[k] = live[k] ? nx[k] : 0.0;
        fetchF(t - 1, nx);
        ss_fwd_step<NPL>(c, x, ev, out, S);
#pragma unroll
        for (int k = 0; k < NPL; ++k) x[k] = out[k] + cur[k];
    }
    double *Wout = a.Y + (size_t)ce * Mp * Mp;
    double *gout = a.Z + (size_t)ce * Mp * Mp;
    double out[NPL], S;
    ss_fwd_step<NPL>(c, x, ev, out, S);
#pragma unroll
    for (int k = 0; k < NPL; ++k) {
        if (live[k]) Wout[(size_t)st[k] * Mp + rc] = x[k];
        if (st[k] == rc) gout[rc] = out[k];
    }
}

struct GPiece {
    long long row;
    int q;
    int o0, len, span;
    int kid, es;
};
struct GTile { int es, cnt; int pid[16]; };

struct PieceArgs {
    int M, Mp, npieces, ntiles;
    const GPiece *pieces;
    const GTile *tiles;
    const double *Xs, *Ys;
    const double *dsc;
    const double *PT, *Pinvrm;
    const double *cs;
    const double *l2d;
    float *pvf;
    double *pvb;
    double *pgam;
};

__global__ __launch_bounds__(256) void k_piece_rowsums(int Ke, int Mp, const double *__restrict__ PT, const double *__restrict__ Pinvrm,
                                                       double *__restrict__ cs, const double *__restrict__ dsc, double *__restrict__ l2d) {
    const int idx = blockIdx.x * 256 + threadIdx.x;
    if (idx < Ke * Mp) l2d[idx] = log2(fabs(dsc[idx]));
    if (idx >= Ke * 2 * Mp) return;
    const int a = idx % Mp, dir = (idx / Mp) & 1, e = idx / (2 * Mp);
    const double *src = (dir ? Pinvrm : PT) + (size_t)e * Mp * Mp + (size_t)a * Mp;
    double acc = 0.0;
    for (int i = 0; i < Mp; ++i) acc += src[i];
    cs[idx] = acc;
}

__global__ __launch_bounds__(256) void k_piece_vectors(PieceArgs a) {
    extern __shared__ __attribute__((aligned(16))) double pv_sm[];
    const int Mp = a.Mp, M = a.M, LDX = Mp + 4;
    const int lane = threadIdx.x & 63, wv = threadIdx.x >> 6;
    const int n = lane & 15, kq = lane >> 4;
    double *sX = pv_sm + (size_t)wv * 16 * LDX;
    const int nunits = 2 * ((a.ntiles + 3) / 4);
    for (int unit = blockIdx.x; unit < nunits; unit += gridDim.x) {
        const int dir = unit & 1;
        const int tile = 4 * (unit >> 1) + wv;
        const bool have = tile < a.ntiles;
        const GTile &tl = a.tiles[min(tile, a.ntiles - 1)];
        const int es = ss_uni(tl.es), cnt = have ? ss_uni(tl.cnt) : 0;
        const int pid = tl.pid[max(0, min(n, cnt - 1))];
        const GPiece pc = a.pieces[pid];
        const int kpow = dir ? pc.span - pc.o0 - pc.len : pc.o0;
        const bool need = n < cnt && kpow > 0;
        const double *X = (dir ? a.Ys : a.Xs) + (size_t)pc.q * Mp;
        const double *dsc = a.dsc + (size_t)es * Mp;
// ... 191 lines not shown
```

### smcpp_amd/csrc/engine_plans.hpp

```cpp
template <auto KERNEL>
static void lds_limit_once() {
    static bool once = false;
    if (!once) { HIPCHK(hipFuncSetAttribute((const void *)KERNEL, hipFuncAttributeMaxDynamicSharedMemorySize, 160 * 1024)); once = true; }
}

template <int MT_, bool TAB_, bool RERUN_, bool HOT2_>
static void launch_chain_coop2_tt(bool fwd, const ChainArgs &a, const CoopArgs &ca, size_t shm, hipStream_t s) {
    if (fwd) {
        lds_limit_once<k_fwd_coop2<MT_, TAB_, RERUN_, HOT2_>>();
        hipLaunchKernelGGL((k_fwd_coop2<MT_, TAB_, RERUN_, HOT2_>), dim3(a.nchunks), dim3(MT_ * 4), shm, s, a, ca);
    } else {
        lds_limit_once<k_bwd_coop2<MT_, TAB_, RERUN_, HOT2_>>();
        hipLaunchKernelGGL((k_bwd_coop2<MT_, TAB_, RERUN_, HOT2_>), dim3(a.nchunks), dim3(MT_ * 4), shm, s, a, ca);
    }
}
template <int MT_, bool TAB_>
static void launch_chain_power_t(bool fwd, const ChainArgs &a, const CoopArgs &ca, size_t shm, hipStream_t s) {
    if (fwd) {
        lds_limit_once<k_fwd_coop2<MT_, TAB_, false, false, true>>();
        hipLaunchKernelGGL((k_fwd_coop2<MT_, TAB_, false, false, true>), dim3(a.nchunks), dim3(MT_ * 4), shm, s, a, ca);
    } else {
        lds_limit_once<k_bwd_coop2<MT_, TAB_, false, false, true>>();
        hipLaunchKernelGGL((k_bwd_coop2<MT_, TAB_, false, false, true>), dim3(a.nchunks), dim3(MT_ * 4), shm, s, a, ca);
    }
// ... 288 lines not shown
            }
        }
        if (first_round) HIPCHK(hipEventRecord(ev[EV_BWD_START], dual ? sb : s));
        if (!bdone) {
            a.changed = d_changed_b.p;
            for (; launched_b < want_b; ++launched_b) {
                set_variant(launched_b);
                if (!(chain_mode == 4 && launch_chain_lock(false, Mp, a, sb)) &&
                    !(chain_mode == 3 && launch_chain_big(false, Mp, a, bargs, sb)) &&
                    !(chain_mode == 2 && launch_chain_coop(false, Mp, a, cargs, tab_c, shm_c, sb)))
                    throw std::runtime_error("internal: no dense chain kernel for this number of hidden states");
            }
        }
        HIPCHK(hipGetLastError());
        if (first_round && dual) HIPCHK(hipEventRecord(ev[EV_FWD_END], s));
        HIPCHK(hipMemcpyAsync(chf, d_changed_f.p, sizeof(int) * (max_pass + 1), hipMemcpyDeviceToHost, s));
        HIPCHK(hipMemcpyAsync(chb, d_changed_b.p, sizeof(int) * (max_pass + 1), hipMemcpyDeviceToHost, sb));
        if (dual) {
            HIPCHK(hipEventRecord(ev[EV_CHAIN_SYNC], sb));
            HIPCHK(hipStreamWaitEvent(s, ev[EV_CHAIN_SYNC], 0));
        }
        HIPCHK(hipEventRecord(ev[EV_CHAINS_END], s));
        if (first_round && !save_gamma) enqueue_stats();
        else stats_enqueued = false;
        HIPCHK(hipStreamSynchronize(s));
        if (dual) HIPCHK(hipStreamSynchronize(sb));
        first_round = false;
        fq = first_quiet(chf, launched_f);
        bq = first_quiet(chb, launched_b);
        fdone = fq >= 0 || launched_f >= max_pass;
        bdone = bq >= 0 || launched_b >= max_pass;
        if (fdone && bdone) break;
        stats_enqueued = false;
        if (!fdone) want_f = std::min(max_pass, launched_f + 4);
        if (!bdone) want_b = std::min(max_pass, launched_b + 4);
    }
    chains_dual = dual;
    if (a.dbg) {
        long long h[16];
        HIPCHK(hipMemcpy(h, d_dbg.p, sizeof(h), hipMemcpyDeviceToHost));
        for (int w = 0; w < 4; ++w)
            fprintf(stderr, "[cycles] fwd wg1 wave%d: loop %lld, end-barrier %lld, mid-barrier %lld, rows %lld\n", w, h[4 * w], h[4 * w + 1], h[4 * w + 2], h[4 * w + 3]);
    }
    if (fq < 0 || bq < 0) { stats_enqueued = false; throw std::runtime_error("chunk-boundary iteration did not converge"); }
    last_fwd_passes = fq;
    last_bwd_passes = bq;
    if (warm_start && chain_mode == 2 && Mp <= 64) {
        const size_t nel = chunks.size() * (size_t)Mp;
        d_warm_f.alloc(nel); d_warm_b.alloc(nel);
        HIPCHK(hipMemcpyAsync(d_warm_f.p, d_ends_f.p + (size_t)((launched_f - 1) & 1) * nel, nel * sizeof(float),
                              hipMemcpyDeviceToDevice, s));
        HIPCHK(hipMemcpyAsync(d_warm_b.p, d_ends_b.p + (size_t)((launched_b - 1) & 1) * nel, nel * sizeof(double),
                              hipMemcpyDeviceToDevice, s));
        warm_valid = true;
    }
}

static bool ss_generators(int M, int MS, const double *Tm, std::vector<double> &gen, double &c0_out) {
    const double c0 = 1e-5 / (double)(M + 1);
    const double tol = 1e-11;
    std::vector<double> d(M), g(M, 0.0), a(M, 0.0), b(M, 0.0);
    for (int j = 0; j < M; ++j) d[j] = Tm[(size_t)j * M + j];
    for (int j = 0; j + 1 < M; ++j) {
        g[j] = Tm[(size_t)(M - 1) * M + j];
        b[j] = Tm[(size_t)j * M + j + 1] - c0;
    }
    for (int i = 1; i < M; ++i) {
        const double *row = Tm + (size_t)i * M;
        for (int j = 0; j < i && j + 1 < M; ++j)
            if (!(std::fabs(row[j] - g[j]) <= tol * std::fabs(g[j]))) return false;
    }
    {
        std::vector<int> ib(M, 0);
        std::vector<double> best(M, -1.0);
        for (int i = 0; i + 2 < M; ++i) {
            const double *row = Tm + (size_t)i * M;
            for (int j = std::max(1, i + 1); j + 1 < M; ++j)
                if (row[j] > best[j]) { best[j] = row[j]; ib[j] = i; }
        }
        for (int j = 1; j + 1 < M; ++j) {
            const double den = Tm[(size_t)ib[j] * M + j] - c0;
            a[j] = den > 0.0 ? (Tm[(size_t)ib[j] * M + j + 1] - c0) / den : 0.0;
        }
    }
    for (int i = 0; i + 1 < M; ++i) {
        double v = b[i];
        for (int j = i + 1; j < M; ++j) {
            const double t = Tm[(size_t)i * M + j];
            if (!(std::fabs(c0 + v - t) <= tol * std::fabs(t)) || !(t > 0.0)) return false;
            v *= a[j];
        }
    }
    for (int j = 0; j < M; ++j)
        if (!(d[j] > 0.0) || !std::isfinite(a[j]) || !std::isfinite(b[j])) return false;
    c0_out = c0;
    gen.assign((size_t)10 * MS, 0.0);
    double *f_dc = &gen[0], *f_g = f_dc + MS, *f_cg = f_g + MS, *f_b = f_cg + MS, *f_a = f_b + MS, *f_d = f_a + MS,
           *b_dc = f_d + MS, *b_g = b_dc + MS, *b_b = b_g + MS, *b_a = b_b + MS;
    for (int j = 0; j < M; ++j) {
        f_dc[j] = d[j] - c0; f_g[j] = g[j]; f_cg[j] = c0 - g[j]; f_b[j] = b[j]; f_a[j] = a[j]; f_d[j] = d[j];
        const int p = MS - 1 - j;
        b_dc[p] = d[j] - c0; b_g[p] = g[j]; b_b[p] = b[j]; b_a[p] = a[j];
    }
    return true;
}

static bool ss_generators_from_tgen(int M, int MS, const smcpp_host::TransitionGenJac &tj, std::vector<double> &gen, double &c0_out) {
    if (!tj.ok || tj.M != M || (int)tj.ed.size() != std::max(0, M - 1) || (int)tj.pf.size() != M || (int)tj.W.size() != M) return false;
    const double beta = 1e-5, c0 = beta / (double)(M + 1), om = 1.0 - beta;
    auto mix = [&](double raw) { return std::max(raw, 1e-20) * om; };
    std::vector<double> d(M), g(M, 0.0), a(M, 0.0), b(M, 0.0), below(M, 0.0), above(M + 1, 0.0);
    for (int j = 1; j < M; ++j) below[j] = below[j - 1] + tj.ed[j - 1];
    for (int c = M - 1; c >= 1; --c) above[c] = above[c + 1] + tj.W[c];
    for (int j = 0; j + 1 < M; ++j) {
        g[j] = mix(tj.ed[j]) + c0;
        b[j] = mix(tj.pf[j] * tj.W[j + 1]);
    }
    for (int j = 1; j + 1 < M; ++j) a[j] = tj.W[j] > 0.0 ? tj.W[j + 1] / tj.W[j] : 0.0;
    for (int j = 0; j < M; ++j) d[j] = mix(1.0 - (below[j] + tj.pf[j] * above[j + 1])) + c0;
    for (int j = 0; j < M; ++j)
        if (!(d[j] > 0.0) || !std::isfinite(a[j]) || !std::isfinite(b[j]) || !(b[j] >= 0.0) || (j + 1 < M && !(g[j] > 0.0))) return false;
    c0_out = c0;
    gen.assign((size_t)10 * MS, 0.0);
    double *f_dc = &gen[0], *f_g = f_dc + MS, *f_cg = f_g + MS, *f_b = f_cg + MS, *f_a = f_b + MS, *f_d = f_a + MS,
           *b_dc = f_d + MS, *b_g = b_dc + MS, *b_b = b_g + MS, *b_a = b_b + MS;
    for (int j = 0; j < M; ++j) {
        f_dc[j] = d[j] - c0; f_g[j] = g[j]; f_cg[j] = c0 - g[j]; f_b[j] = b[j]; f_a[j] = a[j]; f_d[j] = d[j];
        const int p = MS - 1 - j;
        b_dc[p] = d[j] - c0; b_g[p] = g[j]; b_b[p] = b[j]; b_a[p] = a[j];
    }
    return true;
}

bool smcpp_im::ss_generators_only() {
    if ((T_lazy || T_from_gen) && tgen_valid && ss_generators_from_tgen(M, 64 * NPL, tgen, ss_gen, ss_c0)) {
    } else {
        ensure_T();
        if (!ss_generators(M, 64 * NPL, T.data(), ss_gen, ss_c0)) return false;
    }
    return true;
}

bool smcpp_im::ss_extract_generators() {
    if (!ss_generators_only()) return false;
    if (!E_on_dev) for (const Group &gr : groups) {
        if (ss_hybrid && gr.span > ss_hyb_th) continue;
        double mn = 1.0;
        for (int i = 0; i < M; ++i) mn = std::min(mn, E[(size_t)gr.kid * M + i]);
        if (!(mn > 0.0) || (double)gr.span * std::log(mn) < -450.0) return false;
    }
    return true;
}

template <int NPL_, bool HYB_, bool ALL_, bool H32_ = false>
static void launch_chain_ss_tt(const SsArgs &a, int ntasks, size_t shm, hipStream_t s, int wgw) {
    lds_limit_once<k_chain_ss<NPL_, HYB_, ALL_, H32_>>();
    hipLaunchKernelGGL((k_chain_ss<NPL_, HYB_, ALL_, H32_>), dim3(ntasks / wgw), dim3(64 * wgw), shm, s, a);
}
template <int NPL_, bool HYB_>
static void launch_chain_ss_t(const SsArgs &a, int ntasks, size_t shm, hipStream_t s, int wgw) {
    const bool h32_off = opt().off(smcpp_opt::O_SS_H32);
    if (NPL_ == 1 && !HYB_ && a.K <= a.nlds && a.Mp <= 32 && !h32_off) launch_chain_ss_tt<NPL_, HYB_, true, NPL_ == 1 && !HYB_>(a, ntasks, shm, s, wgw);
    else if (a.K <= a.nlds) launch_chain_ss_tt<NPL_, HYB_, true>(a, ntasks, shm, s, wgw);
    else launch_chain_ss_tt<NPL_, HYB_, false>(a, ntasks, shm, s, wgw);
}
static void launch_chain_ss(int npl, const SsArgs &a, int ntasks, size_t shm, hipStream_t s, int wgw = 4) {
    switch (npl) {
        case 1: if (a.hyb_th != 0x7fffffff) launch_chain_ss_t<1, true>(a, ntasks, shm, s, wgw); else launch_chain_ss_t<1, false>(a, ntasks, shm, s, 4); break;
        case 2: launch_chain_ss_t<2, false>(a, ntasks, shm, s, 4); break;
        case 3: launch_chain_ss_t<3, false>(a, ntasks, shm, s, 4); break;
        case 4: launch_chain_ss_t<4, false>(a, ntasks, shm, s, 4); break;
        case 8: launch_chain_ss_t<8, false>(a, ntasks, shm, s, 4); break;
        case 16: launch_chain_ss_t<16, false>(a, ntasks, shm, s, 4); break;
        default: throw std::runtime_error("unsupported number of hidden states");
    }
}


void smcpp_im::ss_launch_passes(int upto) {
    const size_t shm = (size_t)ss_nlds * 64 * NPL * sizeof(double) + ss_tab_bytes();
    for (; ss_launched < upto; ++ss_launched) {
        const int p = ss_launched;
        const bool lf = p < ss_light_f, lb = p < ss_light_b;
        ss_args.pass = p;
        ss_args.mode_f = lf ? 2 : p == 0 ? 0 : 1;
        ss_args.mode_b = lb ? 2 : p == 0 ? 0 : 1;
        ss_args.full_f = (p > 0 && p == ss_light_f) ? 1 : 0;
        ss_args.full_b = (p > 0 && p == ss_light_b) ? 1 : 0;
        launch_chain_ss(NPL, ss_args, (int)ss_tasks.size(), shm, stream, ss_wg_waves);
    }
    HIPCHK(hipGetLastError());
}

void smcpp_im::ss_launch_initial() {
    hipStream_t s = stream;
    const int MS = 64 * NPL;
    std::vector<float> &pi_f = hs_pi_f;
    if (pi_f.size() != (size_t)Mp) pi_f.assign(Mp, 0.f);
    for (int i = 0; i < M; ++i) pi_f[i] = (float)pi[i];
    const size_t need = 12 * 256 + pi_f.size() * 4 + ss_gen.size() * 8 + (size_t)K * MS * 8;
    pre_stage.reset(need);
    if (need > pre_cap) {
        if (d_pre) (void)hipFree(d_pre);
        pre_cap = need + need / 4;
        HIPCHK(hipMalloc((void **)&d_pre, pre_cap));
        smcpp_opt::poison(d_pre, pre_cap, __LINE__, __FILE__, true);
    }
    size_t off = 0;
    auto put = [&](const void *src, size_t bytes) {
        off = (off + 255) & ~(size_t)255;
        if (src) std::memcpy(pre_stage.base + off, src, bytes);
        char *dp = d_pre + off;
        off += bytes;
        return dp;
    };
    SsArgs &a = ss_args;
    a = SsArgs();
    a.M = M; a.Mp = Mp; a.nchunks = (int)chunks.size(); a.pass = 0; a.K = K; a.nlds = ss_nlds;
    a.chunks = d_chunks.p; a.rowdesc = d_rowdesc_ss.p + ROWDESC_PAD;
    a.chunks_b = d_chunks_b.p; a.nchunks_b = (int)chunks_b.size(); a.tasks = d_tasks.p;
    a.pi_f = reinterpret_cast<const float *>(put(pi_f.data(), pi_f.size() * 4));
    const double *gd = reinterpret_cast<const double *>(put(ss_gen.data(), ss_gen.size() * 8));
    a.f_dc = gd; a.f_g = gd + MS; a.f_cg = gd + 2 * MS; a.f_b = gd + 3 * MS; a.f_a = gd + 4 * MS; a.f_d = gd + 5 * MS;
    a.b_dc = gd + 6 * MS; a.b_g = gd + 7 * MS; a.b_b = gd + 8 * MS; a.b_a = gd + 9 * MS;
    a.c0 = ss_c0;
    if (E_on_dev) a.E = dprep->d_Es.p;
    else {
        const size_t eoff = (off + 255) & ~(size_t)255;
        double *he = reinterpret_cast<double *>(pre_stage.base + eoff);
        std::memset(he, 0, (size_t)K * MS * 8);
        for (int k = 0; k < K; ++k)
            std::memcpy(he + (size_t)ss_slot_of_key[k] * MS, &E[(size_t)k * M], sizeof(double) * M);
        a.E = reinterpret_cast<const double *>(put(nullptr, (size_t)K * MS * 8));
    }
    a.alpha = d_alpha.p; a.beta = d_beta.p; a.cnorm = d_cnorm.p;
    a.ends_f = d_ends_f.p; a.used_f = d_used_f.p; a.ends_b = d_ends_b.p; a.used_b = d_used_b.p;
    {
        if (h_flags_cap < 4 * (max_pass + 1)) {
            if (h_flags) (void)hipHostFree(h_flags);
            h_flags_cap = 4 * (max_pass + 1);
            HIPCHK(hipHostMalloc((void **)&h_flags, sizeof(int) * h_flags_cap, hipHostMallocCoherent | hipHostMallocMapped));
            d_flags_view = nullptr;
        }
        if (!d_flags_view) HIPCHK(hipHostGetDevicePointer((void **)&d_flags_view, h_flags, 0));
        if (!h_done) {
            HIPCHK(hipHostMalloc((void **)&h_done, 64, hipHostMallocCoherent | hipHostMallocMapped));
            *h_done = 0;
            HIPCHK(hipHostGetDevicePointer((void **)&d_done_view, h_done, 0));
        }
        std::memset(h_flags, 0, sizeof(int) * h_flags_cap);
    }
    a.changed_f = d_flags_view; a.changed_b = d_flags_view + (max_pass + 1);
    a.endchg_f = d_flags_view + 2 * (max_pass + 1); a.endchg_b = d_flags_view + 3 * (max_pass + 1);
    a.eps_f = eps_f; a.eps_b = eps_b; a.full_f = a.full_b = 0;
    {
        const bool mixed_on = !opt().off(smcpp_opt::O_SS_MIXED);
        a.mixed = (mixed_on && NPL == 1 && !ss_hybrid) ? 1 : 0;
    }
    if (ss_hybrid) {
        a.hyb_th = ss_hyb_th; a.Ke = Ke; a.hot_ek = std::max(0, hot_eig); a.dirsplit = ss_dirsplit ? 1 : 0;
        a.nk_lds = ss_nk_lds;
        for (int e = 0; e < 4; ++e) { a.key_of_slot[e] = ss_ekey_of_slot[e]; a.slot_of_key[e] = ss_eslot_of_key[e]; }
        a.Pinvrm = d_Pinvrm.p; a.Prm = d_Prm.p; a.PinvT = d_PinvT.p; a.PT = d_PT.p; a.dsc = d_dsc.p;
    }
    {
        long long pos = 0;
        const int ef = opt().i(smcpp_opt::O_SS_LIGHT_F, -1), eb = opt().i(smcpp_opt::O_SS_LIGHT_B, -1);
        pos = ss_positions / std::max<size_t>(1, chunks.size());
        const long long pos_b = ss_positions / std::max<size_t>(1, chunks_b.size());
        auto pick = [&](double hist, long long p_) { return p_ <= 0 || (double)p_ > 1.5 * hist ? 0 : std::min(4, (int)std::ceil(hist / (double)p_)); };
        ss_light_f = ef >= 0 ? ef : pick(2800.0, pos);
        ss_light_b = eb >= 0 ? eb : pick(3900.0, pos_b);
        if (chunks.size() <= (size_t)n_contigs) ss_light_f = 0;
        if (chunks_b.size() <= (size_t)n_contigs) ss_light_b = 0;
    }
    if (ss_hybrid) ss_light_f = ss_light_b = 0;
    const bool use_halo = ss_halo && !(warm_start && ss_warm_valid) && chunks.size() > (size_t)n_contigs && chunks_b.size() > (size_t)n_contigs;
    if (use_halo) ss_light_f = ss_light_b = 0;
    a.halo = use_halo ? 1 : 0;
    ss_pass0 = 0;
    if (warm_start && ss_warm_valid && chunks.size() > (size_t)n_contigs && chunks_b.size() > (size_t)n_contigs) {
        ss_pass0 = ss_warm_parity == 0 ? 1 : 2;
        ss_light_f = ss_pass0 + std::max(0, ss_light_f - 1);
        ss_light_b = ss_pass0 + std::max(0, ss_light_b - 1);
    }
    ss_warm_valid = false;
    a.dbg = nullptr;
    if (opt().has(smcpp_opt::O_DEBUG_CYCLES)) { d_dbg.alloc(16); d_dbg.zero(s); a.dbg = d_dbg.p; }
    HIPCHK(hipMemcpyAsync(d_pre, pre_stage.base, off, hipMemcpyHostToDevice, s));
    HIPCHK(hipEventRecord(ev[EV_FIRST_PASS], s));
    ss_launched = ss_pass0;
    const bool cert_launch = opt().on(smcpp_opt::O_SS_CERT_PASS);
    const int want = std::min(max_pass, std::max(ss_pass0 + (last_ss_passes > 0 ? last_ss_passes + (cert_launch || ss_need_cert_pass ? 1 : 0) : 6),
                                                 std::max(ss_light_f, ss_light_b) + 2));
    ss_launch_passes(want);
}

bool smcpp_im::wait_done(int epoch) {
    const auto t0 = std::chrono::steady_clock::now();
    unsigned n = 0;
    while (__atomic_load_n(h_done, __ATOMIC_ACQUIRE) != epoch) {
#if defined(__x86_64__) || defined(__i386__)
        __builtin_ia32_pause();
#else
        std::this_thread::yield();
#endif
        if ((++n & 0x3fff) == 0 && std::chrono::duration<double>(std::chrono::steady_clock::now() - t0).count() > 5.0) {
            HIPCHK(hipStreamSynchronize(stream));
            return __atomic_load_n(h_done, __ATOMIC_ACQUIRE) == epoch;
        }
    }
    return true;
}

void smcpp_im::run_chains_ss() {
// ... 612 lines not shown
```

### smcpp_amd/csrc/engine_rccl.hpp

```cpp
extern "C" {
struct ncclUniqueIdBlob { char b[128]; };
static void check_rc(int rc) { if (rc) throw std::runtime_error(g_err); }
struct RcclDirect {
    void *lib = nullptr;
    void *comm = nullptr;
    int world = 1, rank = 0;
    int (*get_uid)(void *) = nullptr;
    int (*init_rank)(void **, int, ncclUniqueIdBlob, int) = nullptr;
    int (*all_reduce)(const void *, void *, size_t, int, int, void *, hipStream_t) = nullptr;
    int (*destroy)(void *) = nullptr;
    const char *(*err_string)(int) = nullptr;
    DevBuf<double> buf;
    long n = 0;
    double *h_val = nullptr, *d_val_view = nullptr;
    int *h_flag = nullptr, *d_flag_view = nullptr;
    int epoch = 0;
    bool reduced_in_buf = false;
};
static void *rccl_handle(const char *libpath) {
    static std::mutex mu;
    static std::map<std::string, void *> handles;
    const std::string key = libpath && *libpath ? libpath : "librccl.so.1";
    std::lock_guard<std::mutex> lk(mu);
    auto it = handles.find(key);
// ... 18 lines not shown
        return p;
    };
    r.get_uid = reinterpret_cast<int (*)(void *)>(sym("ncclGetUniqueId"));
    r.init_rank = reinterpret_cast<int (*)(void **, int, ncclUniqueIdBlob, int)>(sym("ncclCommInitRank"));
    r.all_reduce = reinterpret_cast<int (*)(const void *, void *, size_t, int, int, void *, hipStream_t)>(sym("ncclAllReduce"));
    r.destroy = reinterpret_cast<int (*)(void *)>(sym("ncclCommDestroy"));
    r.err_string = reinterpret_cast<const char *(*)(int)>(sym("ncclGetErrorString"));
}
static void rccl_check(const RcclDirect &r, int rc, const char *what) {
    if (rc != 0) throw std::runtime_error(std::string("RCCL: ") + what + ": " + (r.err_string ? r.err_string(rc) : "error"));
}
int smcpp_rccl_unique_id(const char *libpath, char *out128) {
    API_BEGIN
    RcclDirect r;
    rccl_resolve(r, libpath);
    ncclUniqueIdBlob id;
    rccl_check(r, r.get_uid(&id), "ncclGetUniqueId");
    std::memcpy(out128, id.b, 128);
    API_END
}
int smcpp_rccl_init(smcpp_im *im, const char *libpath, const char *id128, int rank, int world) {
    API_BEGIN
    if (im->rccl) throw std::runtime_error("smcpp_rccl_init: already initialised");
    HIPCHK(hipSetDevice(im->device));
    std::unique_ptr<RcclDirect> r(new RcclDirect());
    rccl_resolve(*r, libpath);
    ncclUniqueIdBlob id;
    std::memcpy(id.b, id128, 128);
    r->world = world; r->rank = rank;
    rccl_check(*r, r->init_rank(&r->comm, world, id, rank), "ncclCommInitRank");
    HIPCHK(hipHostMalloc((void **)&r->h_val, 64, hipHostMallocCoherent | hipHostMallocMapped));
    HIPCHK(hipHostGetDevicePointer((void **)&r->d_val_view, r->h_val, 0));
    HIPCHK(hipHostMalloc((void **)&r->h_flag, 64, hipHostMallocCoherent | hipHostMallocMapped));
    *r->h_flag = 0;
    HIPCHK(hipHostGetDevicePointer((void **)&r->d_flag_view, r->h_flag, 0));
    im->rccl = r.release();
    API_END
}
int smcpp_rccl_destroy(smcpp_im *im) {
    API_BEGIN
    if (im->rccl) {
        HIPCHK(hipSetDevice(im->device));
        (void)hipStreamSynchronize(im->stream);
        if (im->rccl->comm && im->rccl->destroy) (void)im->rccl->destroy(im->rccl->comm);
        if (im->rccl->h_val) (void)hipHostFree(im->rccl->h_val);
        if (im->rccl->h_flag) (void)hipHostFree(im->rccl->h_flag);
        delete im->rccl;
        im->rccl = nullptr;
    }
    API_END
}
int smcpp_rccl_exchange(smcpp_im *im, double *loglik_sum) {
    API_BEGIN
    RcclDirect *r = im->rccl;
    if (!r) throw std::runtime_error("smcpp_rccl_exchange: smcpp_rccl_init has not been called");
    long n = 0;
    check_rc(smcpp_pack_stats(im, nullptr, &n, 0));
    if (r->n != n) { r->buf.alloc((size_t)n); r->n = n; }
    check_rc(smcpp_pack_stats(im, r->buf.p, nullptr, 2));
    rccl_check(*r, r->all_reduce(r->buf.p, r->buf.p, (size_t)n,  8,  0, r->comm, im->stream), "ncclAllReduce");
    const int ep = ++r->epoch;
    hipLaunchKernelGGL(k_publish_scalar, dim3(1), dim3(1), 0, im->stream, (const double *)r->buf.p, r->d_val_view, r->d_flag_view, ep);
    HIPCHK(hipGetLastError());
    const auto t0 = std::chrono::steady_clock::now();
    unsigned spins = 0;
    while (__atomic_load_n(r->h_flag, __ATOMIC_ACQUIRE) != ep) {
#if defined(__x86_64__) || defined(__i386__)
        __builtin_ia32_pause();
#else
        std::this_thread::yield();
#endif
        if ((++spins & 0x3fff) == 0 && std::chrono::duration<double>(std::chrono::steady_clock::now() - t0).count() > 30.0) {
            HIPCHK(hipStreamSynchronize(im->stream));
            break;
        }
    }
    *loglik_sum = *r->h_val;
    r->reduced_in_buf = true;
    API_END
}
int smcpp_rccl_unpack(smcpp_im *im) {
    API_BEGIN
    RcclDirect *r = im->rccl;
    if (!r || !r->reduced_in_buf) throw std::runtime_error("smcpp_rccl_unpack: no reduced statistics to hand over");
    check_rc(smcpp_unpack_stats(im, r->buf.p, r->n, 1));
    r->reduced_in_buf = false;
    API_END
}
int smcpp_rccl_fetch(smcpp_im *im, double *out, long n) {
    API_BEGIN
    RcclDirect *r = im->rccl;
    if (!r || n != r->n) throw std::runtime_error("smcpp_rccl_fetch: wrong length");
    HIPCHK(hipSetDevice(im->device));
    HIPCHK(hipStreamSynchronize(im->stream));
    HIPCHK(hipMemcpy(out, r->buf.p, sizeof(double) * n, hipMemcpyDeviceToHost));
    API_END
}

int smcpp_set_chunking(smcpp_im *im, int rows_per_chunk, double eps_alpha, double eps_beta) {
    API_BEGIN
    HIPCHK(hipSetDevice(im->device));
    if (eps_alpha > 0) im->eps_f = (float)eps_alpha;
    if (eps_beta > 0) im->eps_b = eps_beta;
    if (rows_per_chunk != im->user_rows_per_chunk) {
        im->user_rows_per_chunk = rows_per_chunk;
        im->warm_valid = false;
        im->make_chunks();
        im->upload_chunk_state();
        im->setup_power();
        im->last_fwd_passes = im->last_bwd_passes = 0;
    }
    API_END
}

int smcpp_last_timing(smcpp_im *im, double out[9]) {
    API_BEGIN im->resolve_timing(); std::memcpy(out, im->timing, sizeof(double) * 9); API_END
}

int smcpp_last_host_timing(smcpp_im *im, double out[4]) {
    API_BEGIN std::memcpy(out, im->host_timing, sizeof(double) * 4); API_END
}

void *smcpp_stream(smcpp_im *im) { return (void *)im->stream; }

int smcpp_host_chunk_counts(int n_contigs, const long long *cost, const int *rows, long long nslots, long long floor_cost, int *out) {
    API_BEGIN
    if (n_contigs <= 0 || nslots <= 0) throw std::runtime_error("smcpp_host_chunk_counts: empty input");
    const std::vector<long long> c(cost, cost + n_contigs);
    const std::vector<int> r(rows, rows + n_contigs);
    const std::vector<int> ncs = ss_chunk_counts(c, r, nslots, floor_cost);
    std::copy(ncs.begin(), ncs.end(), out);
    API_END
}

int smcpp_chain_mode(smcpp_im *im) { return im ? (im->ss_static ? (im->ss_hybrid ? 6 : 5) : im->chain_mode) : -1; }

int smcpp_debug_chunks(smcpp_im *im, int backward, int cap, int *out) {
    if (!im) return -1;
    const std::vector<Chunk> &v = backward ? im->chunks_b : im->chunks;
    for (size_t j = 0; j < v.size() && (long long)j < (long long)cap && out; ++j) {
        const Chunk &ch = v[j];
        const int t[5] = {ch.contig, ch.r0, ch.r1, ch.h0, ch.h1};
        std::copy(t, t + 5, out + 5 * j);
    }
    return (int)v.size();
}

void smcpp_reload_options(void) { smcpp_opt::reload(); }

int smcpp_describe(smcpp_im *im, char *buf, int cap) {
    std::string s = "{";
    s += smcpp_opt::describe_options();
    if (im) {
        char t[1024];
        const int fam = im->ss_static ? (im->ss_hybrid ? 6 : 5) : im->chain_mode;
        snprintf(t, sizeof t,
                 ", \"plan\": {\"chain_family\": %d, \"scan_chains\": %s, \"hybrid_rows\": %s, \"states\": %d, \"states_padded\": %d, "
                 "\"states_per_lane\": %d, \"keys\": %d, \"eigen_keys\": %d, \"rows\": %lld, \"positions\": %lld, \"max_span\": %d, "
                 "\"chunks_forward\": %zu, \"chunks_backward\": %zu, \"wavefronts_per_simd\": %d, \"halo_pass\": %s, "
                 "\"light_passes_forward\": %d, \"light_passes_backward\": %d, \"float_scans_in_stored_passes\": %s, "
                 "\"passes_to_certificate\": %d, \"passes_launched\": %d, \"certificate_pass_launched_up_front\": %s, "
                 "\"save_gamma\": %s, \"eigen_free_statistics\": %s, \"per_row_gamma\": \"%s\", \"long_rows_cut\": %s, \"warm_start\": %s, \"host_threads\": %d}",
                 fam, im->ss_static ? "true" : "false", im->ss_hybrid ? "true" : "false", im->M, im->Mp, im->NPL, im->K, im->Ke,
                 (long long)(im->total_rows - im->n_contigs), (long long)im->ss_positions, im->ss_max_span, im->chunks.size(),
                 im->chunks_b.size(), im->ss_wpc, (im->ss_static && im->ss_args.halo) ? "true" : "false", im->ss_light_f, im->ss_light_b,
                 (im->ss_static && im->ss_args.mixed) ? "true" : "false", im->last_ss_passes, im->ss_launched,
                 (opt().on(smcpp_opt::O_SS_CERT_PASS) || im->ss_need_cert_pass) ? "true" : "false", im->save_gamma ? "true" : "false",
                 im->eigfree ? "true" : "false", !im->save_gamma ? "none" : im->eigfree ? "scan steps" : im->stats_plan.gamma_form == StatsPlan::GAMMA_PIECES ? "eigen-power pieces + scan steps" : "eigensystem", im->split_spans ? "true" : "false",
                 im->warm_start ? "true" : "false", omp_get_max_threads());
        s += t;
        const StatsPlan &p = im->stats_plan;
        static const char *const stream[] = {"main", "second", "third", "high priority"}, *const rank[] = {"per slab", "teams", "wide"};
        static const char *const eigen[] = {"none", "fold on the scans", "fold on the matrix cores", "generation 2", "classic"};
        static const char *const gsum[] = {"one pass", "own stream", "span > 1 tail", "span-1 branch"};
        static const char *const gamma[] = {"none", "scan steps", "eigen-power pieces + scan steps", "eigensystem batches", "eigensystem rows"};
        snprintf(t, sizeof t,
                 ", \"statistics\": {\"span_gt1_stream\": \"%s\", \"span1_stream\": \"%s\", \"gamma_sums_stream\": \"%s\", "
                 "\"loglik_stream\": \"%s\", \"per_row_gamma_stream\": \"%s\", \"span1_form\": \"%s\", \"rank_update\": \"%s\", "
                 "\"eigen\": \"%s\", \"span_gt1_rank_early\": %s, \"gamma_sums_reduced\": \"%s\", \"per_row_gamma\": \"%s\", "
                 "\"per_row_gamma_beside\": %s}",
                 stream[p.span_gt1], stream[p.span1], stream[p.gsum], stream[p.loglik], stream[p.gamma], p.s1_one_pass ? "one pass" : "two kernels",
                 rank[p.rank], eigen[p.eigen], p.rank_early ? "true" : "false", gsum[p.gsum_at], gamma[p.gamma_form], p.gamma_beside ? "true" : "false");
        s += p.resolved ? t : ", \"statistics\": null";
        static const char *const route[] = {"none", "device", "host"};
        s += std::string(", \"q_route\": \"") + route[im->q_route] + "\"";
    }
    s += "}";
    if (buf && cap > 0) {
        const size_t n = std::min(s.size(), (size_t)cap - 1);
        std::memcpy(buf, s.data(), n);
        buf[n] = 0;
    }
    return (int)s.size();
}

static int ss_debug_apply(int M, const double *T, int nvec, const double *x, const double *e, double *out_f, double *out_b, int float_scans);
int smcpp_debug_ss_apply(int M, const double *T, int nvec, const double *x, const double *e, double *out_f, double *out_b) {
    API_BEGIN
    return ss_debug_apply(M, T, nvec, x, e, out_f, out_b, 0);
    API_END
}
int smcpp_debug_ss_apply_float_scans(int M, const double *T, int nvec, const double *x, const double *e, double *out_f, double *out_b) {
    API_BEGIN
    if (M > 64) throw std::runtime_error("the all-float scans hold one state per lane: M <= 64");
    return ss_debug_apply(M, T, nvec, x, e, out_f, out_b, 1);
    API_END
}
static int ss_debug_apply(int M, const double *T, int nvec, const double *x, const double *e, double *out_f, double *out_b, int float_scans) {
    {
    const int NPL = M > 512 ? 16 : M > 256 ? 8 : (M + 63) / 64, MS = 64 * NPL;
    if (M > 1024) throw std::runtime_error("unsupported number of hidden states");
    std::vector<double> gen;
    double c0 = 0.0;
    if (!ss_generators(M, MS, T, gen, c0)) return 2;
    std::vector<double> hx((size_t)nvec * MS, 0.0), he((size_t)nvec * MS, 0.0);
    for (int v = 0; v < nvec; ++v) {
        std::memcpy(&hx[(size_t)v * MS], x + (size_t)v * M, sizeof(double) * M);
        std::memcpy(&he[(size_t)v * MS], e + (size_t)v * M, sizeof(double) * M);
    }
    DevBuf<double> dg, dx, de, df, db;
    hipStream_t s = nullptr;
    dg.upload(gen, s); dx.upload(hx, s); de.upload(he, s);
    df.alloc(hx.size()); db.alloc(hx.size());
    SsArgs a = SsArgs();
    a.M = M;
    const double *gd = dg.p;
    a.f_dc = gd; a.f_g = gd + MS; a.f_cg = gd + 2 * MS; a.f_b = gd + 3 * MS; a.f_a = gd + 4 * MS; a.f_d = gd + 5 * MS;
    a.b_dc = gd + 6 * MS; a.b_g = gd + 7 * MS; a.b_b = gd + 8 * MS; a.b_a = gd + 9 * MS;
    a.c0 = c0;
    if (float_scans && M <= 32) hipLaunchKernelGGL((k_ss_apply<1, true, true>), dim3(nvec), dim3(64), 0, s, a, (const double *)dx.p, (const double *)de.p, df.p, db.p, nvec);
    else if (float_scans) hipLaunchKernelGGL((k_ss_apply<1, true, false>), dim3(nvec), dim3(64), 0, s, a, (const double *)dx.p, (const double *)de.p, df.p, db.p, nvec);
    else switch (NPL) {
        case 1: hipLaunchKernelGGL(k_ss_apply<1>, dim3(nvec), dim3(64), 0, s, a, (const double *)dx.p, (const double *)de.p, df.p, db.p, nvec); break;
        case 2: hipLaunchKernelGGL(k_ss_apply<2>, dim3(nvec), dim3(64), 0, s, a, (const double *)dx.p, (const double *)de.p, df.p, db.p, nvec); break;
        case 3: hipLaunchKernelGGL(k_ss_apply<3>, dim3(nvec), dim3(64), 0, s, a, (const double *)dx.p, (const double *)de.p, df.p, db.p, nvec); break;
        case 4: hipLaunchKernelGGL(k_ss_apply<4>, dim3(nvec), dim3(64), 0, s, a, (const double *)dx.p, (const double *)de.p, df.p, db.p, nvec); break;
        case 8: hipLaunchKernelGGL(k_ss_apply<8>, dim3(nvec), dim3(64), 0, s, a, (const double *)dx.p, (const double *)de.p, df.p, db.p, nvec); break;
        default: hipLaunchKernelGGL(k_ss_apply<16>, dim3(nvec), dim3(64), 0, s, a, (const double *)dx.p, (const double *)de.p, df.p, db.p, nvec); break;
    }
    HIPCHK(hipGetLastError());
    std::vector<double> hf(hx.size()), hb(hx.size());
    HIPCHK(hipMemcpy(hf.data(), df.p, hf.size() * sizeof(double), hipMemcpyDeviceToHost));
    HIPCHK(hipMemcpy(hb.data(), db.p, hb.size() * sizeof(double), hipMemcpyDeviceToHost));
    for (int v = 0; v < nvec; ++v) {
        std::memcpy(out_f + (size_t)v * M, &hf[(size_t)v * MS], sizeof(double) * M);
        std::memcpy(out_b + (size_t)v * M, &hb[(size_t)v * MS], sizeof(double) * M);
    }
    }
    return 0;
}


int smcpp_device(smcpp_im *im) { return im ? im->device : -1; }
int smcpp_set_debug(smcpp_im *im, int on) { API_BEGIN im->debug = on != 0; API_END }
int smcpp_get_debug(smcpp_im *im) { return im && im->debug ? 1 : 0; }

void smcpp_set_num_threads(int k) { if (k > 0) omp_set_num_threads(k); }

int smcpp_host_set_csfs_direct(int on) {
    const int prev = smcpp_host::csfs_direct_flag();
    smcpp_host::csfs_direct_flag() = on != 0;
    return prev;
}

}
```

### smcpp_amd/csrc/kernels.hpp

```cpp
#pragma once
#include <hip/hip_runtime.h>
#include <stdint.h>

namespace smcpp_dev {

typedef double f64x4 __attribute__((ext_vector_type(4)));

struct Chunk {
    long long base;
    int r0, r1;
    int contig;
    int first;
    int last;
    int pad;
    int h0 = 0, h1 = 0;
};

struct RowInfo {
    int kid;
    int gid;
};
#define SMCPP_GID(ge) ((ge) & 0xFFFFF)
#define SMCPP_ES(ge) ((ge) >> 20)

// ... 931 lines not shown
    const double *beta;
    const double *w1;
    const double *cnorm;
    const double *E;
    const double *Xs, *Ys;
    double *part;
    double *gpart;
    const int2 *teams;
};

template <int MODE, bool TEAM = false>
__global__ __launch_bounds__(TEAM ? 256 : 64) __attribute__((amdgpu_waves_per_eu(2))) void k_rank_acc(AccArgs a) {
    const int lane = threadIdx.x & 63, wv = threadIdx.x >> 6;
    const int m = lane & 15, qd = lane >> 4;
    int slab_id = blockIdx.x;
    bool have = true;
    if (TEAM) {
        const int2 tm = a.teams[blockIdx.x];
        const int wu = __builtin_amdgcn_readfirstlane(wv);
        have = wu < tm.y;
        slab_id = tm.x + (have ? wu : 0);
    }
    const Slab sl = a.slabs[slab_id];
    const int Mp = a.Mp;
    const int jb = (blockIdx.y / a.NB) * 64, kb = (blockIdx.y % a.NB) * 64;
    f64x4 acc[4][4];
#pragma unroll
    for (int i = 0; i < 4; ++i)
#pragma unroll
        for (int j = 0; j < 4; ++j) acc[i][j] = (f64x4){0, 0, 0, 0};
    if (TEAM && !have) {
    } else if (MODE == 0 || MODE == 2 || MODE == 3) {
        const int last = sl.end - 1;
        auto fetch_pk = [&](int r0) {
            const int r = r0 + qd;
            int2 pk;
            if (MODE == 0) pk = a.permk[min(r, last)];
            else { pk.x = a.perm[min(r, last)]; pk.y = MODE == 3 ? sl.aux : 0; }
            pk.x = (r <= last) ? pk.x : -1;
            return pk;
        };
        struct Ops { double w; float ap[4], an[4]; double bp[4], ep[4]; bool valid; };
        int jc[4], kc[4];
        bool jv[4], kv[4];
        const int j0 = jb + 4 * m, k0 = kb + 4 * m;
        const int j0c = j0 < Mp ? j0 : 0, k0c = k0 < Mp ? k0 : 0;
#pragma unroll
        for (int t = 0; t < 4; ++t) {
            jv[t] = j0 < Mp; kv[t] = k0 < Mp;
            jc[t] = j0c + t; kc[t] = k0c + t;
        }
        double ekc[4] = {1.0, 1.0, 1.0, 1.0}, gsum[4] = {0.0, 0.0, 0.0, 0.0};
        if (MODE == 3) {
#pragma unroll
            for (int t = 0; t < 4; ++t) ekc[t] = a.E[(size_t)sl.aux * Mp + kc[t]];
        }
        auto fetch_ops = [&](const int2 pk) {
            Ops o;
            o.valid = pk.x >= 0;
            const size_t row = (size_t)(sl.base + (o.valid ? pk.x : 1));
            const bool inl = a.NB == 1;
            o.w = inl ? a.cnorm[row] : a.w1[row];
            const float *ap = a.alpha + (row - 1) * Mp;
            const double *bp = a.beta + row * Mp;
            const double *ep = a.E + (size_t)pk.y * Mp;
            const float4 a4 = *reinterpret_cast<const float4 *>(ap + j0c);
            const double4 b4 = *reinterpret_cast<const double4 *>(bp + k0c);
            o.ap[0] = a4.x; o.ap[1] = a4.y; o.ap[2] = a4.z; o.ap[3] = a4.w;
            o.bp[0] = b4.x; o.bp[1] = b4.y; o.bp[2] = b4.z; o.bp[3] = b4.w;
            if (MODE == 0) {
                const double4 e4 = *reinterpret_cast<const double4 *>(ep + k0c);
                o.ep[0] = e4.x; o.ep[1] = e4.y; o.ep[2] = e4.z; o.ep[3] = e4.w;
            } else {
#pragma unroll
                for (int t = 0; t < 4; ++t) o.ep[t] = MODE == 3 ? ekc[t] : 1.0;
            }
            if (inl) {
                const float4 n4 = *reinterpret_cast<const float4 *>(ap + Mp + k0c);
                o.an[0] = n4.x; o.an[1] = n4.y; o.an[2] = n4.z; o.an[3] = n4.w;
            } else {
#pragma unroll
                for (int t = 0; t < 4; ++t) o.an[t] = 0.f;
            }
            return o;
        };
        auto consume = [&](const Ops &cur) {
            double xa[4], yb[4];
            double wgt = cur.w;
            if (a.NB == 1) {
                double pp = 0.0;
#pragma unroll
                for (int t = 0; t < 4; ++t) pp += kv[t] ? (double)cur.an[t] * cur.bp[t] : 0.0;
                const double psum = row16_sum(pp);
                wgt = 1.0 / (cur.w * psum);
                if (MODE == 3) {
                    const double ip = 1.0 / psum;
#pragma unroll
                    for (int t = 0; t < 4; ++t)
                        gsum[t] += (cur.valid && kv[t]) ? (double)cur.an[t] * cur.bp[t] * ip : 0.0;
                }
            }
#pragma unroll
            for (int t = 0; t < 4; ++t) {
                xa[t] = (cur.valid && jv[t]) ? wgt * (double)cur.ap[t] : 0.0;
                yb[t] = kv[t] ? cur.bp[t] * cur.ep[t] : 0.0;
            }
#pragma unroll
            for (int i = 0; i < 4; ++i)
#pragma unroll
                for (int j = 0; j < 4; ++j)
                    acc[i][j] = __builtin_amdgcn_mfma_f64_16x16x4f64(xa[i], yb[j], acc[i][j], 0, 0, 0);
        };
        int2 pk1 = fetch_pk(sl.start);
        Ops cur = fetch_ops(pk1);
        pk1 = fetch_pk(sl.start + 4);
        Ops nx1 = fetch_ops(pk1);
        pk1 = fetch_pk(sl.start + 8);
        for (int r0 = sl.start; r0 < sl.end; r0 += 4) {
            const int2 pk2 = fetch_pk(r0 + 12);
            const Ops nxt = fetch_ops(pk1);
            consume(cur);
            cur = nx1;
            nx1 = nxt;
            pk1 = pk2;
        }
        if (MODE == 3) {
#pragma unroll
            for (int t = 0; t < 4; ++t) {
                double v = gsum[t];
                v += __shfl_xor(v, 16);
                v += __shfl_xor(v, 32);
                if (qd == 0 && k0 < Mp) a.gpart[(size_t)slab_id * Mp + k0 + t] = v;
            }
        }
    } else {
        for (int r0 = sl.start; r0 < sl.end; r0 += 4) {
            const int r = r0 + qd;
            const bool valid = r < sl.end;
            double xa[4], yb[4];
            const size_t row = (size_t)(valid ? r : sl.start);
#pragma unroll
            for (int t = 0; t < 4; ++t) {
                const int j = jb + 16 * t + m, k = kb + 16 * t + m;
                xa[t] = (valid && j < Mp) ? a.Xs[row * Mp + j] : 0.0;
                yb[t] = (valid && k < Mp) ? a.Ys[row * Mp + k] : 0.0;
            }
#pragma unroll
            for (int i = 0; i < 4; ++i)
#pragma unroll
                for (int j = 0; j < 4; ++j)
                    acc[i][j] = __builtin_amdgcn_mfma_f64_16x16x4f64(xa[i], yb[j], acc[i][j], 0, 0, 0);
        }
    }
    if (TEAM) {
        __shared__ double red[2][64 * 64];
        if (wv >= 2) {
#pragma unroll
            for (int i = 0; i < 4; ++i)
#pragma unroll
                for (int j = 0; j < 4; ++j)
#pragma unroll
                    for (int rg = 0; rg < 4; ++rg) red[wv - 2][((i * 4 + j) * 4 + rg) * 64 + lane] = acc[i][j][rg];
        }
        __syncthreads();
        if (wv < 2) {
#pragma unroll
            for (int i = 0; i < 4; ++i)
#pragma unroll
                for (int j = 0; j < 4; ++j)
#pragma unroll
                    for (int rg = 0; rg < 4; ++rg) acc[i][j][rg] += red[wv][((i * 4 + j) * 4 + rg) * 64 + lane];
        }
        __syncthreads();
        if (wv == 1) {
#pragma unroll
            for (int i = 0; i < 4; ++i)
#pragma unroll
                for (int j = 0; j < 4; ++j)
#pragma unroll
                    for (int rg = 0; rg < 4; ++rg) red[0][((i * 4 + j) * 4 + rg) * 64 + lane] = acc[i][j][rg];
        }
        __syncthreads();
        if (wv != 0) return;
#pragma unroll
        for (int i = 0; i < 4; ++i)
#pragma unroll
            for (int j = 0; j < 4; ++j)
#pragma unroll
                for (int rg = 0; rg < 4; ++rg) acc[i][j][rg] += red[0][((i * 4 + j) * 4 + rg) * 64 + lane];
    }
    double *out = a.part + (size_t)blockIdx.x * Mp * Mp;
    if (MODE != 1) {
        const int col = kb + 4 * m;
#pragma unroll
        for (int i = 0; i < 4; ++i)
#pragma unroll
            for (int rg = 0; rg < 4; ++rg) {
                const int row = jb + 4 * (qd + 4 * rg) + i;
                if (row < Mp && col < Mp)
                    *reinterpret_cast<double4 *>(out + (size_t)row * Mp + col) = make_double4(acc[i][0][rg], acc[i][1][rg], acc[i][2][rg], acc[i][3][rg]);
            }
        return;
    }
#pragma unroll
    for (int i = 0; i < 4; ++i)
#pragma unroll
        for (int j = 0; j < 4; ++j)
#pragma unroll
            for (int rg = 0; rg < 4; ++rg) {
                const int row = jb + 16 * i + qd + 4 * rg;
                const int col = kb + 16 * j + m;
                if (row < Mp && col < Mp) out[(size_t)row * Mp + col] = acc[i][j][rg];
            }
}


constexpr int RW_R = 16;
constexpr int RW_XS = 256 + 16;
constexpr int RW_YS = 128 + 16;
constexpr size_t RW_LDS = 2 * (size_t)RW_R * (RW_XS + RW_YS) * sizeof(double);

template <int MODE, int NWV>
__global__ __launch_bounds__(64 * NWV) void k_rank_acc_wide(AccArgs a) {
    constexpr int XT = 16 / NWV;
    constexpr int RPT = RW_R / NWV;
    static_assert(MODE == 0 || MODE == 2, "span-1 rows (0) or the eigen-free span > 1 rows (2)");
    extern __shared__ double rw_lds[];
    const int lane = threadIdx.x & 63;
    const int wv = __builtin_amdgcn_readfirstlane((int)(threadIdx.x >> 6));
    const int m = lane & 15, qd = lane >> 4;
    const int Mp = a.Mp;
    const int nby = (Mp + 127) / 128;
    const int jb = ((int)blockIdx.y / nby) * 256, kb = ((int)blockIdx.y % nby) * 128;
    int first = blockIdx.x, cnt = 1;
    if (a.teams) { const int2 tm = a.teams[blockIdx.x]; first = tm.x; cnt = tm.y; }
    const Slab s_first = a.slabs[first], s_last = a.slabs[first + cnt - 1];
    const int R0 = s_first.start, R1 = s_last.end;
    const long long base = s_first.base;
    auto sXb = [&](int buf) { return rw_lds + buf * (RW_R * (RW_XS + RW_YS)); };
    const bool wave_on = jb + 16 * XT * wv < Mp;
    f64x4 acc[XT][8];
#pragma unroll
    for (int i = 0; i < XT; ++i)
#pragma unroll
        for (int j = 0; j < 8; ++j) acc[i][j] = (f64x4){0, 0, 0, 0};
    const bool xin = jb + 4 * lane < Mp, yin = kb + 2 * lane < Mp;
    const int xcol = xin ? jb + 4 * lane : 0, ycol = yin ? kb + 2 * lane : 0;
    struct Stage { float4 al[RPT]; double2 be[RPT]; double2 em[RPT]; double w[RPT]; };
    auto fetch_idx = [&](int r0, int2 (&pk)[RPT]) {
#pragma unroll
        for (int i = 0; i < RPT; ++i) {
            const int r = r0 + wv + NWV * i;
            const int rc = min(r, R1 - 1);
            if (MODE == 0) pk[i] = a.permk[rc];
            else { pk[i].x = a.perm[rc]; pk[i].y = 0; }
            if (r >= R1) pk[i].x = -1;
        }
    };
    auto fetch_ops = [&](const int2 (&pk)[RPT], Stage &o) {
#pragma unroll
        for (int i = 0; i < RPT; ++i) {
            const bool valid = pk[i].x >= 0;
            const size_t row = (size_t)(base + (valid ? pk[i].x : 1));
            const double w = a.w1[row];
            o.w[i] = valid ? w : 0.0;
            o.al[i] = *reinterpret_cast<const float4 *>(a.alpha + (row - 1) * Mp + xcol);
            o.be[i] = *reinterpret_cast<const double2 *>(a.beta + row * Mp + ycol);
            if (MODE == 0) o.em[i] = *reinterpret_cast<const double2 *>(a.E + (size_t)pk[i].y * Mp + ycol);
        }
    };
    auto stash = [&](const Stage &o, int buf) {
        double *sX = sXb(buf), *sY = sXb(buf) + RW_R * RW_XS;
#pragma unroll
        for (int i = 0; i < RPT; ++i) {
            const int rr = wv + NWV * i;
            const double w = xin ? o.w[i] : 0.0;
            double *px = sX + rr * RW_XS + 4 * lane;
            *reinterpret_cast<double2 *>(px) = make_double2(w * (double)o.al[i].x, w * (double)o.al[i].y);
            *reinterpret_cast<double2 *>(px + 2) = make_double2(w * (double)o.al[i].z, w * (double)o.al[i].w);
            double2 y = o.be[i];
            if (MODE == 0) { y.x *= o.em[i].x; y.y *= o.em[i].y; }
            if (!yin) y = make_double2(0.0, 0.0);
            *reinterpret_cast<double2 *>(sY + rr * RW_YS + 2 * lane) = y;
        }
    };
    auto compute = [&](int buf) {
        const double *sX = sXb(buf) + 16 * XT * wv + m, *sY = sXb(buf) + RW_R * RW_XS + m;
#pragma unroll
        for (int kk = 0; kk < RW_R / 4; ++kk) {
            const double *px = sX + (4 * kk + qd) * RW_XS, *py = sY + (4 * kk + qd) * RW_YS;
            double xa[XT], yb[8];
#pragma unroll
            for (int i = 0; i < XT; ++i) xa[i] = px[16 * i];
#pragma unroll
            for (int j = 0; j < 8; ++j) yb[j] = py[16 * j];
#pragma unroll
            for (int i = 0; i < XT; ++i)
#pragma unroll
                for (int j = 0; j < 8; ++j)
                    acc[i][j] = __builtin_amdgcn_mfma_f64_16x16x4f64(xa[i], yb[j], acc[i][j], 0, 0, 0);
        }
    };
    if (R1 > R0) {
        const int nst = (R1 - R0 + RW_R - 1) / RW_R;
        int2 pk[RPT];
        Stage st;
        fetch_idx(R0, pk);
        fetch_ops(pk, st);
        fetch_idx(R0 + RW_R, pk);
        stash(st, 0);
        __syncthreads();
        for (int s = 0; s < nst; ++s) {
            fetch_ops(pk, st);
            fetch_idx(R0 + RW_R * (s + 2), pk);
            if (wave_on) compute(s & 1);
            stash(st, (s + 1) & 1);
            __syncthreads();
        }
    }
    if (!wave_on) return;
    double *out = a.part + (size_t)blockIdx.x * Mp * Mp;
#pragma unroll
    for (int i = 0; i < XT; ++i)
#pragma unroll
        for (int j = 0; j < 8; ++j)
#pragma unroll
            for (int rg = 0; rg < 4; ++rg) {
                const int row = jb + 16 * XT * wv + 16 * i + qd + 4 * rg;
                const int col = kb + 16 * j + m;
                if (row < Mp && col < Mp) out[(size_t)row * Mp + col] = acc[i][j][rg];
            }
}


struct PackArgs {
    int M, Mp, K, Kg, n_contigs;
    const double *loglik;
    const double *gamma0;
    const double *xisum;
    const double *gsum;
    const unsigned char *present;
    const int *g2l;
    double *out;
};

__global__ __launch_bounds__(256) void k_pack_stats(PackArgs a) {
    const long n = 1 + a.M + (long)a.M * a.M + (long)a.Kg * a.M;
    const long idx = (long)blockIdx.x * 256 + threadIdx.x;
    if (idx >= n) return;
    double acc = 0.0;
    if (idx == 0) {
        for (int c = 0; c < a.n_contigs; ++c) acc += a.loglik[c];
    } else if (idx < 1 + a.M) {
        const int i = (int)idx - 1;
        for (int c = 0; c < a.n_contigs; ++c) acc += a.gamma0[(size_t)c * a.Mp + i];
    } else if (idx < 1 + a.M + (long)a.M * a.M) {
        const long e = idx - 1 - a.M;
        const int i = (int)(e / a.M), j = (int)(e % a.M);
        for (int c = 0; c < a.n_contigs; ++c) acc += a.xisum[((size_t)c * a.Mp + i) * a.Mp + j];
    } else {
        const long e = idx - 1 - a.M - (long)a.M * a.M;
        const int kg = (int)(e / a.M), i = (int)(e % a.M);
        const int k = a.g2l[kg];
        if (k >= 0)
            for (int c = 0; c < a.n_contigs; ++c)
// ... 697 lines not shown
```

Baseline: 1114.

## Add all-lanes-live chain kernel variant specialised on halo/full flags for M=64

Adds a LIVE template path to the scan-chain kernel, used when M equals Mp equals 64 with mixed scans. It removes per-lane liveness masks and turns the full/halo runtime flags into compile-time constants, so dead branches drop out of the forward/backward loops. The f64-to-f32 conversion and initial multiply now sit inside the DPP scan asm, and light-scan helpers get fused variants. In the team accumulator the final LDS reduction is folded into the output stores. These changes add kernel instantiations and code size, which may cost compile time and instruction cache.

Measured after the change: 1085. -2.6%, worse.

```diff
diff --git a/smcpp_amd/csrc/chains_ss.hpp b/smcpp_amd/csrc/chains_ss.hpp
--- a/smcpp_amd/csrc/chains_ss.hpp
+++ b/smcpp_amd/csrc/chains_ss.hpp
@@ -156,11 +156,13 @@
 
 #define SS_D_ " row_mask:0xf bank_mask:0xf bound_ctrl:1\n"
 template <bool H32>
-__device__ __forceinline__ void ss_x_scan_fwd(float &z, float &s, float &zp, float &tot, const float (&lv)[6], float m1, float m2,
+__device__ __forceinline__ void ss_x_scan_fwd(double x, float bf, float &zp, float &tot, const float (&lv)[6], float m1, float m2,
                                               float m3, float bg, float c0) {
-    float t1, t2, t3;
+    float t1, t2, t3, z, s;
     if (H32) {
-        asm volatile("s_nop 1\n"
+        asm volatile("v_cvt_f32_f64_e32 %1, %13\n"
+                     "v_mul_f32_e32 %0, %14, %1\n"
+                     "s_nop 0\n"
                      "v_add_f32_dpp %1, %1, %1 row_shl:1" SS_D_ "v_fmac_f32_dpp %0, %0, %5 row_shr:1" SS_D_ "s_nop 0\n"
                      "v_add_f32_dpp %1, %1, %1 row_shl:2" SS_D_ "v_fmac_f32_dpp %0, %0, %6 row_shr:2" SS_D_ "s_nop 0\n"
                      "v_add_f32_dpp %1, %1, %1 row_shl:4" SS_D_ "v_fmac_f32_dpp %0, %0, %7 row_shr:4" SS_D_ "s_nop 0\n"
@@ -174,11 +176,13 @@
                      "v_mov_b32_dpp %2, %0 wave_shr:1" SS_D_
                      "v_fmac_f32_e32 %2, %11, %1\n"
                      "v_fmac_f32_e32 %2, %3, %12\n"
-                     : "+v"(z), "+v"(s), "=&v"(zp), "=&s"(tot), "=&s"(t1)
-                     : "v"(lv[0]), "v"(lv[1]), "v"(lv[2]), "v"(lv[3]), "v"(lv[4]), "v"(m1), "v"(bg), "v"(c0));
+                     : "=&v"(z), "=&v"(s), "=&v"(zp), "=&s"(tot), "=&s"(t1)
+                     : "v"(lv[0]), "v"(lv[1]), "v"(lv[2]), "v"(lv[3]), "v"(lv[4]), "v"(m1), "v"(bg), "v"(c0), "v"(x), "v"(bf));
         return;
     }
-    asm volatile("s_nop 1\n"
+    asm volatile("v_cvt_f32_f64_e32 %1, %18\n"
+                 "v_mul_f32_e32 %0, %19, %1\n"
+                 "s_nop 0\n"
                  "v_add_f32_dpp %1, %1, %1 row_shl:1" SS_D_ "v_fmac_f32_dpp %0, %0, %7 row_shr:1" SS_D_ "s_nop 0\n"
                  "v_add_f32_dpp %1, %1, %1 row_shl:2" SS_D_ "v_fmac_f32_dpp %0, %0, %8 row_shr:2" SS_D_ "s_nop 0\n"
                  "v_add_f32_dpp %1, %1, %1 row_shl:4" SS_D_ "v_fmac_f32_dpp %0, %0, %9 row_shr:4" SS_D_ "s_nop 0\n"
@@ -196,15 +200,18 @@
                  "v_fmac_f32_e32 %2, %16, %1\n"
                  "s_nop 0\n"
                  "v_fmac_f32_e32 %2, %3, %17\n"
-                 : "+v"(z), "+v"(s), "=&v"(zp), "=&s"(tot), "=&s"(t1), "=&s"(t2), "=&s"(t3)
-                 : "v"(lv[0]), "v"(lv[1]), "v"(lv[2]), "v"(lv[3]), "v"(lv[4]), "v"(lv[5]), "v"(m1), "v"(m2), "v"(m3), "v"(bg), "v"(c0));
+                 : "=&v"(z), "=&v"(s), "=&v"(zp), "=&s"(tot), "=&s"(t1), "=&s"(t2), "=&s"(t3)
+                 : "v"(lv[0]), "v"(lv[1]), "v"(lv[2]), "v"(lv[3]), "v"(lv[4]), "v"(lv[5]), "v"(m1), "v"(m2), "v"(m3), "v"(bg), "v"(c0),
+                   "v"(x), "v"(bf));
 }
 template <bool H32>
-__device__ __forceinline__ void ss_x_scan_bwd(float &v, float &f, float &gs, float &tot, const float (&lv)[6], float c15, float c31,
+__device__ __forceinline__ void ss_x_scan_bwd(double w0, float gf, float &f, float &gs, float &tot, const float (&lv)[6], float c15, float c31,
                                               float m1, float m2, float m3, float b, float c0) {
-    float t1, t2, t3, vp;
+    float t1, t2, t3, vp, v;
     if (H32) {
-        asm volatile("s_nop 1\n"
+        asm volatile("v_cvt_f32_f64_e32 %0, %15\n"
+                     "v_mul_f32_e32 %2, %16, %0\n"
+                     "s_nop 0\n"
                      "v_add_f32_dpp %1, %0, %0 row_shr:1" SS_D_ "v_add_f32_dpp %2, %2, %2 row_shl:1" SS_D_ "v_fmac_f32_dpp %0, %0, %6 row_shr:1" SS_D_
                      "v_add_f32_dpp %1, %1, %1 row_shr:2" SS_D_ "v_add_f32_dpp %2, %2, %2 row_shl:2" SS_D_ "v_fmac_f32_dpp %0, %0, %7 row_shr:2" SS_D_
                      "v_add_f32_dpp %1, %1, %1 row_shr:4" SS_D_ "v_add_f32_dpp %2, %2, %2 row_shl:4" SS_D_ "v_fmac_f32_dpp %0, %0, %8 row_shr:4" SS_D_
@@ -217,11 +224,13 @@
                      "v_mov_b32_dpp %4, %0 wave_shr:1" SS_D_
                      "v_fmac_f32_e32 %2, %14, %1\n"
                      "v_fmac_f32_e32 %2, %13, %4\n"
-                     : "+v"(v), "=&v"(f), "+v"(gs), "=&s"(tot), "=&v"(vp), "=&s"(t3)
-                     : "v"(lv[0]), "v"(lv[1]), "v"(lv[2]), "v"(lv[3]), "v"(lv[4]), "v"(c15), "v"(m3), "v"(b), "v"(c0));
+                     : "=&v"(v), "=&v"(f), "=&v"(gs), "=&s"(tot), "=&v"(vp), "=&s"(t3)
+                     : "v"(lv[0]), "v"(lv[1]), "v"(lv[2]), "v"(lv[3]), "v"(lv[4]), "v"(c15), "v"(m3), "v"(b), "v"(c0), "v"(w0), "v"(gf));
         return;
     }
-    asm volatile("s_nop 1\n"
+    asm volatile("v_cvt_f32_f64_e32 %0, %21\n"
+                 "v_mul_f32_e32 %2, %22, %0\n"
+                 "s_nop 0\n"
                  "v_add_f32_dpp %1, %0, %0 row_shr:1" SS_D_ "v_add_f32_dpp %2, %2, %2 row_shl:1" SS_D_ "v_fmac_f32_dpp %0, %0, %8 row_shr:1" SS_D_
                  "v_add_f32_dpp %1, %1, %1 row_shr:2" SS_D_ "v_add_f32_dpp %2, %2, %2 row_shl:2" SS_D_ "v_fmac_f32_dpp %0, %0, %9 row_shr:2" SS_D_
                  "v_add_f32_dpp %1, %1, %1 row_shr:4" SS_D_ "v_add_f32_dpp %2, %2, %2 row_shl:4" SS_D_ "v_fmac_f32_dpp %0, %0, %10 row_shr:4" SS_D_
@@ -240,9 +249,9 @@
                  "v_readlane_b32 %3, %1, 63\n"
                  "v_fmac_f32_e32 %2, %20, %1\n"
                  "v_fmac_f32_e32 %2, %19, %4\n"
-                 : "+v"(v), "=&v"(f), "+v"(gs), "=&s"(tot), "=&v"(vp), "=&s"(t1), "=&s"(t2), "=&s"(t3)
+                 : "=&v"(v), "=&v"(f), "=&v"(gs), "=&s"(tot), "=&v"(vp), "=&s"(t1), "=&s"(t2), "=&s"(t3)
                  : "v"(lv[0]), "v"(lv[1]), "v"(lv[2]), "v"(lv[3]), "v"(lv[4]), "v"(lv[5]), "v"(c15), "v"(c31), "v"(m1), "v"(m2), "v"(m3),
-                   "v"(b), "v"(c0));
+                   "v"(b), "v"(c0), "v"(w0), "v"(gf));
 }
 #undef SS_D_
 
@@ -250,9 +259,8 @@
 __device__ __forceinline__ void ss_fwd_step(const SsFwdC<NPL> &c, const double (&x)[NPL], const double (&e)[NPL],
                                             double (&out)[NPL], double &S) {
     if (MIX && NPL == 1) {
-        float s = (float)x[0];
-        float z = c.bff * s, zp, tot;
-        ss_x_scan_fwd<H32>(z, s, zp, tot, c.lvf, c.m1, c.m2, c.m3, c.bgf, c.c0f);
+        float zp, tot;
+        ss_x_scan_fwd<H32>(x[0], c.bff, zp, tot, c.lvf, c.m1, c.m2, c.m3, c.bgf, c.c0f);
         S = (double)tot;
         out[0] = e[0] * __builtin_fma(c.adg, x[0], (double)zp);
         return;
@@ -297,9 +305,8 @@
                                             double (&out)[NPL], float &Sw) {
     if (MIX && NPL == 1) {
         const double w0 = e[0] * bv[0];
-        float v = (float)w0;
-        float gs = c.gf * v, f;
-        ss_x_scan_bwd<H32>(v, f, gs, Sw, c.lvf, c.c15f, c.c31f, c.m1, c.m2, c.m3, c.bff, c.c0f);
+        float gs, f;
+        ss_x_scan_bwd<H32>(w0, c.gf, f, gs, Sw, c.lvf, c.c15f, c.c31f, c.m1, c.m2, c.m3, c.bff, c.c0f);
         out[0] = __builtin_fma(c.adg, w0, (double)gs);
         return;
     }
@@ -529,18 +536,19 @@
 template <int NPL, bool ALLLDS>
 __device__ __forceinline__ void ss_bwd_light_rows(const SsArgs &a, const double *sE, long long base, int rhi, int rlo, int lane, float (&b)[NPL]);
 
-template <int NPL, bool RERUN, bool HYB, bool ALLLDS, bool MIX = false, bool H32 = false>
+template <int NPL, bool RERUN, bool HYB, bool ALLLDS, bool MIX = false, bool H32 = false, bool LIVE = false, int UNI = -1>
 __device__ __forceinline__ void ss_forward_wave(const SsArgs &a, const double *sE, int c, int lane) {
     constexpr int MS = 64 * NPL;
     const int M = a.M, Mp = a.Mp, pass = a.pass;
     const Chunk ch = ss_uniform_chunk(a.chunks[c]);
+    const bool full = UNI < 0 ? a.full_f != 0 : (UNI & 1) != 0, halo_on = UNI < 0 ? a.halo != 0 : (UNI & 2) != 0;
     float *end_cur = a.ends_f + ((size_t)(pass & 1) * a.nchunks + c) * Mp;
     const float *end_prev = a.ends_f + ((size_t)((pass + 1) & 1) * a.nchunks + c) * Mp;
     int st[NPL];
     bool live[NPL], stor[NPL];
 #pragma unroll
-    for (int k = 0; k < NPL; ++k) { st[k] = lane * NPL + k; live[k] = st[k] < M; stor[k] = st[k] < Mp; }
-    if (RERUN && ch.first && !a.full_f) {
+    for (int k = 0; k < NPL; ++k) { st[k] = lane * NPL + k; live[k] = LIVE || st[k] < M; stor[k] = LIVE || st[k] < Mp; }
+    if (RERUN && ch.first && !full) {
 #pragma unroll
         for (int k = 0; k < NPL; ++k) if (stor[k]) end_cur[st[k]] = end_prev[st[k]];
         return;
@@ -551,7 +559,7 @@
 #pragma unroll
         for (int k = 0; k < NPL; ++k) x[k] = live[k] ? (double)src[st[k]] : 0.0;
     }
-    const bool halo = !RERUN && !HYB && a.halo && ch.h0 < ch.r0;
+    const bool halo = !RERUN && !HYB && halo_on && ch.h0 < ch.r0;
     const int rbeg = halo ? ch.h1 : ch.r0;
     const int jst = ch.r0 - rbeg;
     if (halo && ch.h0 < ch.h1) {
@@ -574,7 +582,7 @@
             }
         }
     }
-    if (RERUN && !a.full_f) {
+    if (RERUN && !full) {
         bool diff = false;
 #pragma unroll
         for (int k = 0; k < NPL; ++k)
@@ -647,7 +655,7 @@
             double xin = x[0] * inv;
             if (j > 0) {
                 const float an = live[0] ? fmaxf((float)xin, flo) : 0.f;
-                if (RERUN && !a.full_f && (j & 15) == 0 && j >= 16) {
+                if (RERUN && !full && (j & 15) == 0 && j >= 16) {
                     bool bad = false;
                     if (live[0]) {
                         const float old = arow[(size_t)j * Mp + st[0]];
@@ -683,7 +691,7 @@
                 an[k] = live[k] ? fmaxf((float)xs, flo) : 0.f;
                 fb[k] = (double)an[k] - xs;
             }
-            if (RERUN && !a.full_f && (j & 15) == 0 && j >= 16) {
+            if (RERUN && !full && (j & 15) == 0 && j >= 16) {
                 bool bad = false;
 #pragma unroll
                 for (int k = 0; k < NPL; ++k)
@@ -763,18 +771,19 @@
     }
 }
 
-template <int NPL, bool RERUN, bool HYB, bool ALLLDS, bool MIX = false, bool H32 = false>
+template <int NPL, bool RERUN, bool HYB, bool ALLLDS, bool MIX = false, bool H32 = false, bool LIVE = false, int UNI = -1>
 __device__ __forceinline__ void ss_backward_wave(const SsArgs &a, const double *sE, int c, int lane) {
     constexpr int MS = 64 * NPL;
     const int M = a.M, Mp = a.Mp, pass = a.pass;
     const Chunk ch = ss_uniform_chunk(a.chunks_b[c]);
+    const bool full = UNI < 0 ? a.full_b != 0 : (UNI & 1) != 0, halo_on = UNI < 0 ? a.halo != 0 : (UNI & 2) != 0;
     double *end_cur = a.ends_b + ((size_t)(pass & 1) * a.nchunks_b + c) * Mp;
     const double *end_prev = a.ends_b + ((size_t)((pass + 1) & 1) * a.nchunks_b + c) * Mp;
     int st[NPL];
     bool live[NPL], stor[NPL];
 #pragma unroll
-    for (int k = 0; k < NPL; ++k) { st[k] = MS - 1 - (lane * NPL + k); live[k] = st[k] < M; stor[k] = st[k] < Mp; }
-    if (RERUN && ch.last && !a.full_b) {
+    for (int k = 0; k < NPL; ++k) { st[k] = MS - 1 - (lane * NPL + k); live[k] = LIVE || st[k] < M; stor[k] = LIVE || st[k] < Mp; }
+    if (RERUN && ch.last && !full) {
 #pragma unroll
         for (int k = 0; k < NPL; ++k) if (stor[k]) end_cur[st[k]] = end_prev[st[k]];
         return;
@@ -786,7 +795,7 @@
 #pragma unroll
         for (int k = 0; k < NPL; ++k) b[k] = live[k] ? (fresh ? 1.0 / (double)M : src[st[k]]) : 0.0;
     }
-    const bool halo = !RERUN && !HYB && a.halo && ch.h0 > ch.r1;
+    const bool halo = !RERUN && !HYB && halo_on && ch.h0 > ch.r1;
     const int rend = halo ? ch.h1 : ch.r1;
     const int jst = rend - ch.r1;
     if (halo && ch.h0 > ch.h1) {
@@ -801,7 +810,7 @@
 #pragma unroll
         for (int k = 0; k < NPL; ++k) b[k] = live[k] ? (double)(bf_[k] * iv) : 0.0;
     }
-    if (RERUN && !a.full_b) {
+    if (RERUN && !full) {
         bool diff = false;
 #pragma unroll
         for (int k = 0; k < NPL; ++k)
@@ -855,7 +864,7 @@
         const int slot_n = __builtin_amdgcn_readlane(dcur.x, (j + 1) & 63) & 0xFFFF;
         double en[NPL];
         ss_emission<NPL, true, ALLLDS>(a, sE, slot_n, lane, en);
-        if (RERUN && !a.full_b && (j & 15) == 0 && j >= 16) {
+        if (RERUN && !full && (j & 15) == 0 && j >= 16) {
             bool bad = false;
 #pragma unroll
             for (int k = 0; k < NPL; ++k)
@@ -971,19 +980,7 @@
 }
 
 #define SS_DPP_ "row_mask:0xf bank_mask:0xf bound_ctrl:1\n"
-template <bool H32>
 __device__ __forceinline__ void ss_light_scan2(float &p, float &z, const float (&lv)[6], float c15, float c31) {
-    if (H32) {
-        asm volatile("s_nop 1\n"
-                     "v_add_f32_dpp %0, %0, %0 row_shr:1 " SS_DPP_ "v_fmac_f32_dpp %1, %1, %2 row_shr:1 " SS_DPP_ "s_nop 0\n"
-                     "v_add_f32_dpp %0, %0, %0 row_shr:2 " SS_DPP_ "v_fmac_f32_dpp %1, %1, %3 row_shr:2 " SS_DPP_ "s_nop 0\n"
-                     "v_add_f32_dpp %0, %0, %0 row_shr:4 " SS_DPP_ "v_fmac_f32_dpp %1, %1, %4 row_shr:4 " SS_DPP_ "s_nop 0\n"
-                     "v_add_f32_dpp %0, %0, %0 row_shr:8 " SS_DPP_ "v_fmac_f32_dpp %1, %1, %5 row_shr:8 " SS_DPP_ "s_nop 0\n"
-                     "v_fmac_f32_dpp %0, %0, %7 row_bcast:15 " SS_DPP_ "v_fmac_f32_dpp %1, %1, %6 row_bcast:15 " SS_DPP_ "s_nop 1\n"
-                     : "+v"(p), "+v"(z)
-                     : "v"(lv[0]), "v"(lv[1]), "v"(lv[2]), "v"(lv[3]), "v"(lv[4]), "v"(c15));
-        return;
-    }
     asm volatile("s_nop 1\n"
                  "v_add_f32_dpp %0, %0, %0 row_shr:1 " SS_DPP_ "v_fmac_f32_dpp %1, %1, %2 row_shr:1 " SS_DPP_ "s_nop 0\n"
                  "v_add_f32_dpp %0, %0, %0 row_shr:2 " SS_DPP_ "v_fmac_f32_dpp %1, %1, %3 row_shr:2 " SS_DPP_ "s_nop 0\n"
@@ -994,19 +991,7 @@
                  : "+v"(p), "+v"(z)
                  : "v"(lv[0]), "v"(lv[1]), "v"(lv[2]), "v"(lv[3]), "v"(lv[4]), "v"(lv[5]), "v"(c15), "v"(c31));
 }
-template <bool H32>
 __device__ __forceinline__ void ss_light_scan3(float &p, float &z, float &f, const float (&lv)[6], float c15, float c31) {
-    if (H32) {
-        asm volatile("s_nop 1\n"
-                     "v_add_f32_dpp %0, %0, %0 row_shr:1 " SS_DPP_ "v_fmac_f32_dpp %1, %1, %3 row_shr:1 " SS_DPP_ "v_add_f32_dpp %2, %2, %2 row_shr:1 " SS_DPP_
-                     "v_add_f32_dpp %0, %0, %0 row_shr:2 " SS_DPP_ "v_fmac_f32_dpp %1, %1, %4 row_shr:2 " SS_DPP_ "v_add_f32_dpp %2, %2, %2 row_shr:2 " SS_DPP_
-                     "v_add_f32_dpp %0, %0, %0 row_shr:4 " SS_DPP_ "v_fmac_f32_dpp %1, %1, %5 row_shr:4 " SS_DPP_ "v_add_f32_dpp %2, %2, %2 row_shr:4 " SS_DPP_
-                     "v_add_f32_dpp %0, %0, %0 row_shr:8 " SS_DPP_ "v_fmac_f32_dpp %1, %1, %6 row_shr:8 " SS_DPP_ "v_add_f32_dpp %2, %2, %2 row_shr:8 " SS_DPP_
-                     "v_fmac_f32_dpp %0, %0, %8 row_bcast:15 " SS_DPP_ "v_fmac_f32_dpp %1, %1, %7 row_bcast:15 " SS_DPP_ "v_fmac_f32_dpp %2, %2, %8 row_bcast:15 " SS_DPP_ "s_nop 1\n"
-                     : "+v"(p), "+v"(z), "+v"(f)
-                     : "v"(lv[0]), "v"(lv[1]), "v"(lv[2]), "v"(lv[3]), "v"(lv[4]), "v"(c15));
-        return;
-    }
     asm volatile("s_nop 1\n"
                  "v_add_f32_dpp %0, %0, %0 row_shr:1 " SS_DPP_ "v_fmac_f32_dpp %1, %1, %3 row_shr:1 " SS_DPP_ "v_add_f32_dpp %2, %2, %2 row_shr:1 " SS_DPP_
                  "v_add_f32_dpp %0, %0, %0 row_shr:2 " SS_DPP_ "v_fmac_f32_dpp %1, %1, %4 row_shr:2 " SS_DPP_ "v_add_f32_dpp %2, %2, %2 row_shr:2 " SS_DPP_
@@ -1017,11 +1002,95 @@
                  : "+v"(p), "+v"(z), "+v"(f)
                  : "v"(lv[0]), "v"(lv[1]), "v"(lv[2]), "v"(lv[3]), "v"(lv[4]), "v"(lv[5]), "v"(c15), "v"(c31));
 }
+template <bool H32>
+__device__ __forceinline__ void ss_light_fwd1(float &x, float &S, float e, float b, float dc, float g, float cg, const float (&lv)[6],
+                                              float c15, float c31) {
+    float p, z, t;
+    if (H32) {
+        asm volatile("v_mul_f32_e32 %2, %6, %0\n"
+                     "v_mul_f32_e32 %3, %7, %0\n"
+                     "v_add_f32_dpp %1, %0, %0 row_shr:1 " SS_DPP_ "v_fmac_f32_dpp %2, %2, %10 row_shr:1 " SS_DPP_ "s_nop 0\n"
+                     "v_add_f32_dpp %1, %1, %1 row_shr:2 " SS_DPP_ "v_fmac_f32_dpp %2, %2, %11 row_shr:2 " SS_DPP_ "s_nop 0\n"
+                     "v_add_f32_dpp %1, %1, %1 row_shr:4 " SS_DPP_ "v_fmac_f32_dpp %2, %2, %12 row_shr:4 " SS_DPP_ "s_nop 0\n"
+                     "v_add_f32_dpp %1, %1, %1 row_shr:8 " SS_DPP_ "v_fmac_f32_dpp %2, %2, %13 row_shr:8 " SS_DPP_ "s_nop 0\n"
+                     "v_fmac_f32_dpp %1, %1, %15 row_bcast:15 " SS_DPP_ "v_fmac_f32_dpp %2, %2, %14 row_bcast:15 " SS_DPP_
+                     "v_readlane_b32 %4, %1, 31\n"
+                     "v_fmac_f32_e32 %3, %9, %1\n"
+                     "v_add_f32_dpp %3, %2, %3 wave_shr:1 " SS_DPP_
+                     "v_fmac_f32_e32 %3, %4, %8\n"
+                     "v_mul_f32_e32 %0, %5, %3\n"
+                     : "+v"(x), "=&v"(p), "=&v"(z), "=&v"(t), "=&s"(S)
+                     : "v"(e), "v"(b), "v"(dc), "v"(g), "v"(cg), "v"(lv[0]), "v"(lv[1]), "v"(lv[2]), "v"(lv[3]), "v"(lv[4]), "v"(c15));
+        return;
+    }
+    asm volatile("v_mul_f32_e32 %2, %6, %0\n"
+                 "v_mul_f32_e32 %3, %7, %0\n"
+                 "v_add_f32_dpp %1, %0, %0 row_shr:1 " SS_DPP_ "v_fmac_f32_dpp %2, %2, %10 row_shr:1 " SS_DPP_ "s_nop 0\n"
+                 "v_add_f32_dpp %1, %1, %1 row_shr:2 " SS_DPP_ "v_fmac_f32_dpp %2, %2, %11 row_shr:2 " SS_DPP_ "s_nop 0\n"
+                 "v_add_f32_dpp %1, %1, %1 row_shr:4 " SS_DPP_ "v_fmac_f32_dpp %2, %2, %12 row_shr:4 " SS_DPP_ "s_nop 0\n"
+                 "v_add_f32_dpp %1, %1, %1 row_shr:8 " SS_DPP_ "v_fmac_f32_dpp %2, %2, %13 row_shr:8 " SS_DPP_ "s_nop 0\n"
+                 "v_fmac_f32_dpp %1, %1, %16 row_bcast:15 " SS_DPP_ "v_fmac_f32_dpp %2, %2, %14 row_bcast:15 " SS_DPP_ "s_nop 0\n"
+                 "v_fmac_f32_dpp %1, %1, %17 row_bcast:31 " SS_DPP_ "v_fmac_f32_dpp %2, %2, %15 row_bcast:31 " SS_DPP_
+                 "v_readlane_b32 %4, %1, 63\n"
+                 "v_fmac_f32_e32 %3, %9, %1\n"
+                 "v_add_f32_dpp %3, %2, %3 wave_shr:1 " SS_DPP_
+                 "v_fmac_f32_e32 %3, %4, %8\n"
+                 "v_mul_f32_e32 %0, %5, %3\n"
+                 : "+v"(x), "=&v"(p), "=&v"(z), "=&v"(t), "=&s"(S)
+                 : "v"(e), "v"(b), "v"(dc), "v"(g), "v"(cg), "v"(lv[0]), "v"(lv[1]), "v"(lv[2]), "v"(lv[3]), "v"(lv[4]), "v"(lv[5]), "v"(c15),
+                   "v"(c31));
+}
+template <bool H32>
+__device__ __forceinline__ void ss_light_bwd1(float &v, float &f, float e, float g, float dc, float c0, float b, const float (&lv)[6],
+                                              float c15, float c31) {
+    float w, p, G;
+    if (H32) {
+        asm volatile("v_mul_f32_e32 %2, %0, %5\n"
+                     "v_mul_f32_e32 %3, %6, %2\n"
+                     "v_mul_f32_e32 %0, %7, %2\n"
+                     "v_add_f32_dpp %1, %2, %2 row_shr:1 " SS_DPP_ "v_add_f32_dpp %3, %3, %3 row_shr:1 " SS_DPP_ "v_fmac_f32_dpp %2, %2, %10 row_shr:1 " SS_DPP_
+                     "v_add_f32_dpp %1, %1, %1 row_shr:2 " SS_DPP_ "v_add_f32_dpp %3, %3, %3 row_shr:2 " SS_DPP_ "v_fmac_f32_dpp %2, %2, %11 row_shr:2 " SS_DPP_
+                     "v_add_f32_dpp %1, %1, %1 row_shr:4 " SS_DPP_ "v_add_f32_dpp %3, %3, %3 row_shr:4 " SS_DPP_ "v_fmac_f32_dpp %2, %2, %12 row_shr:4 " SS_DPP_
+                     "v_add_f32_dpp %1, %1, %1 row_shr:8 " SS_DPP_ "v_add_f32_dpp %3, %3, %3 row_shr:8 " SS_DPP_ "v_fmac_f32_dpp %2, %2, %13 row_shr:8 " SS_DPP_
+                     "v_fmac_f32_dpp %1, %1, %15 row_bcast:15 " SS_DPP_ "v_fmac_f32_dpp %3, %3, %15 row_bcast:15 " SS_DPP_ "v_fmac_f32_dpp %2, %2, %14 row_bcast:15 " SS_DPP_
+                     "v_readlane_b32 %4, %3, 63\n"
+                     "v_fmac_f32_e32 %0, %8, %1\n"
+                     "v_fmac_f32_dpp %0, %2, %9 wave_shr:1 " SS_DPP_
+                     "v_sub_f32_e32 %3, %4, %3\n"
+                     "v_add_f32_e32 %0, %0, %3\n"
+                     : "+v"(v), "=&v"(f), "=&v"(w), "=&v"(p), "=&s"(G)
+                     : "v"(e), "v"(g), "v"(dc), "v"(c0), "v"(b), "v"(lv[0]), "v"(lv[1]), "v"(lv[2]), "v"(lv[3]), "v"(lv[4]), "v"(c15));
+        return;
+    }
+    asm volatile("v_mul_f32_e32 %2, %0, %5\n"
+                 "v_mul_f32_e32 %3, %6, %2\n"
+                 "v_mul_f32_e32 %0, %7, %2\n"
+                 "v_add_f32_dpp %1, %2, %2 row_shr:1 " SS_DPP_ "v_add_f32_dpp %3, %3, %3 row_shr:1 " SS_DPP_ "v_fmac_f32_dpp %2, %2, %10 row_shr:1 " SS_DPP_
+                 "v_add_f32_dpp %1, %1, %1 row_shr:2 " SS_DPP_ "v_add_f32_dpp %3, %3, %3 row_shr:2 " SS_DPP_ "v_fmac_f32_dpp %2, %2, %11 row_shr:2 " SS_DPP_
+                 "v_add_f32_dpp %1, %1, %1 row_shr:4 " SS_DPP_ "v_add_f32_dpp %3, %3, %3 row_shr:4 " SS_DPP_ "v_fmac_f32_dpp %2, %2, %12 row_shr:4 " SS_DPP_
+                 "v_add_f32_dpp %1, %1, %1 row_shr:8 " SS_DPP_ "v_add_f32_dpp %3, %3, %3 row_shr:8 " SS_DPP_ "v_fmac_f32_dpp %2, %2, %13 row_shr:8 " SS_DPP_
+                 "v_fmac_f32_dpp %1, %1, %16 row_bcast:15 " SS_DPP_ "v_fmac_f32_dpp %3, %3, %16 row_bcast:15 " SS_DPP_ "v_fmac_f32_dpp %2, %2, %14 row_bcast:15 " SS_DPP_
+                 "v_fmac_f32_dpp %1, %1, %17 row_bcast:31 " SS_DPP_ "v_fmac_f32_dpp %3, %3, %17 row_bcast:31 " SS_DPP_ "v_fmac_f32_dpp %2, %2, %15 row_bcast:31 " SS_DPP_
+                 "v_readlane_b32 %4, %3, 63\n"
+                 "v_fmac_f32_e32 %0, %8, %1\n"
+                 "v_fmac_f32_dpp %0, %2, %9 wave_shr:1 " SS_DPP_
+                 "v_sub_f32_e32 %3, %4, %3\n"
+                 "v_add_f32_e32 %0, %0, %3\n"
+                 : "+v"(v), "=&v"(f), "=&v"(w), "=&v"(p), "=&s"(G)
+                 : "v"(e), "v"(g), "v"(dc), "v"(c0), "v"(b), "v"(lv[0]), "v"(lv[1]), "v"(lv[2]), "v"(lv[3]), "v"(lv[4]), "v"(lv[5]), "v"(c15),
+                   "v"(c31));
+}
 #undef SS_DPP_
 
 template <int NPL, bool H32 = false>
 __device__ __forceinline__ void ss_fwd_step_f(const SsLightC<NPL> &c, const float (&x)[NPL], const float (&e)[NPL],
                                               float (&out)[NPL], float &S) {
+    if (NPL == 1) {
+        float v = x[0];
+        ss_light_fwd1<H32>(v, S, e[0], c.b[0], c.dc[0], c.g[0], c.cg[0], c.lv, c.c15, c.c31);
+        out[0] = v;
+        return;
+    }
     float lp[NPL], w[NPL];
     lp[0] = x[0];
     w[0] = c.b[0] * x[0];
@@ -1031,13 +1100,9 @@
         w[k] = __builtin_fmaf(c.a[k], w[k - 1], c.b[k] * x[k]);
     }
     float p_ = lp[NPL - 1], z_ = w[NPL - 1];
-    ss_light_scan2<H32>(p_, z_, c.lv, c.c15, c.c31);
-    S = lane_get(p_, H32 ? 31 : 63);
+    ss_light_scan2(p_, z_, c.lv, c.c15, c.c31);
+    S = lane_get(p_, 63);
     const float LIp = dpp0<DPP_WSHR1>(z_);
-    if (NPL == 1) {
-        out[0] = e[0] * __builtin_fmaf(c.dc[0], x[0], __builtin_fmaf(c.g[0], S, __builtin_fmaf(c.cg[0], p_, LIp)));
-        return;
-    }
     const float lex = p_ - lp[NPL - 1];
 #pragma unroll
     for (int k = 0; k < NPL; ++k) {
@@ -1050,6 +1115,13 @@
 template <int NPL, bool H32 = false>
 __device__ __forceinline__ void ss_bwd_step_f(const SsLightC<NPL> &c, const float (&bv)[NPL], const float (&e)[NPL],
                                               float (&out)[NPL], float &Sw) {
+    if (NPL == 1) {
+        float v = bv[0], f;
+        ss_light_bwd1<H32>(v, f, e[0], c.g[0], c.dc[0], c.c0, c.b[0], c.lv, c.c15, c.c31);
+        Sw = lane_get(f, 63);
+        out[0] = v;
+        return;
+    }
     float w[NPL], lg[NPL], u[NPL], lf[NPL];
 #pragma unroll
     for (int k = 0; k < NPL; ++k) w[k] = e[k] * bv[k];
@@ -1063,14 +1135,10 @@
         lf[k] = lf[k - 1] + w[k];
     }
     float p_ = lg[NPL - 1], z_ = u[NPL - 1], f_ = lf[NPL - 1];
-    ss_light_scan3<H32>(p_, z_, f_, c.lv, c.c15, c.c31);
+    ss_light_scan3(p_, z_, f_, c.lv, c.c15, c.c31);
     const float Gtot = lane_get(p_, 63);
     Sw = lane_get(f_, 63);
     const float LIp = dpp0<DPP_WSHR1>(z_);
-    if (NPL == 1) {
-        out[0] = __builtin_fmaf(c.dc[0], w[0], (Gtot - p_) + __builtin_fmaf(c.c0, f_, c.b[0] * LIp));
-        return;
-    }
     const float lexg = p_ - lg[NPL - 1], lexf = f_ - lf[NPL - 1];
 #pragma unroll
     for (int k = 0; k < NPL; ++k) {
@@ -1173,7 +1241,7 @@
     }
 }
 
-template <int NPL, bool ALLLDS, bool H32 = false>
+template <int NPL, bool ALLLDS, bool H32 = false, bool LIVE = false>
 __device__ __forceinline__ void ss_forward_light(const SsArgs &a, const double *sE, int c, int lane) {
     const int M = a.M, Mp = a.Mp, pass = a.pass;
     const Chunk ch = ss_uniform_chunk(a.chunks[c]);
@@ -1181,7 +1249,7 @@
     int st[NPL];
     bool live[NPL], stor[NPL];
 #pragma unroll
-    for (int k = 0; k < NPL; ++k) { st[k] = lane * NPL + k; live[k] = st[k] < M; stor[k] = st[k] < Mp; }
+    for (int k = 0; k < NPL; ++k) { st[k] = lane * NPL + k; live[k] = LIVE || st[k] < M; stor[k] = LIVE || st[k] < Mp; }
     float x[NPL];
     {
         const float *src = (ch.first || pass == 0) ? a.pi_f : a.ends_f + ((size_t)((pass + 1) & 1) * a.nchunks + (c - 1)) * Mp;
@@ -1237,7 +1305,7 @@
     for (int k = 0; k < NPL; ++k) if (stor[k]) end_cur[st[k]] = live[k] ? fmaxf(x[k] * inv, ss_floor_at<NPL>(a, ch.base + ch.r1 + 1)) : 0.f;
 }
 
-template <int NPL, bool ALLLDS, bool H32 = false>
+template <int NPL, bool ALLLDS, bool H32 = false, bool LIVE = false>
 __device__ __forceinline__ void ss_backward_light(const SsArgs &a, const double *sE, int c, int lane) {
     constexpr int MS = 64 * NPL;
     const int M = a.M, Mp = a.Mp, pass = a.pass;
@@ -1246,7 +1314,7 @@
     int st[NPL];
     bool live[NPL], stor[NPL];
 #pragma unroll
-    for (int k = 0; k < NPL; ++k) { st[k] = MS - 1 - (lane * NPL + k); live[k] = st[k] < M; stor[k] = st[k] < Mp; }
+    for (int k = 0; k < NPL; ++k) { st[k] = MS - 1 - (lane * NPL + k); live[k] = LIVE || st[k] < M; stor[k] = LIVE || st[k] < Mp; }
     float b[NPL];
     {
         const bool fresh = ch.last || pass == 0;
@@ -1303,7 +1371,7 @@
     for (int k = 0; k < NPL; ++k) if (stor[k]) end_cur[st[k]] = live[k] ? (double)(b[k] * inv) : 0.0;
 }
 
-template <int NPL, bool HYB, bool ALLLDS, bool H32 = false>
+template <int NPL, bool HYB, bool ALLLDS, bool LIVE = false, bool H32 = false>
 __global__ __launch_bounds__(HYB ? 512 : 256) void k_chain_ss(SsArgs a) {
     constexpr int MS = 64 * NPL;
     extern __shared__ __attribute__((aligned(16))) double ss_lds[];
@@ -1342,6 +1410,15 @@
     const int c = task & 0x3FFFFFFF;
     if (fwd) {
         if (idle_f) return;
+        if (LIVE) {
+            if (a.mode_f == 0) {
+                if (a.halo) ss_forward_wave<NPL, false, HYB, ALLLDS, true, H32, true, 2>(a, ss_lds, c, lane);
+                else ss_forward_wave<NPL, false, HYB, ALLLDS, true, H32, true, 0>(a, ss_lds, c, lane);
+            } else if (a.mode_f == 1) {
+                if (a.full_f) ss_forward_wave<NPL, true, HYB, ALLLDS, true, H32, true, 1>(a, ss_lds, c, lane);
+                else ss_forward_wave<NPL, true, HYB, ALLLDS, true, H32, true, 0>(a, ss_lds, c, lane);
+            } else ss_forward_light<NPL, ALLLDS, H32, true>(a, ss_lds, c, lane);
+        } else
         if (NPL == 1 && !HYB && a.mixed) {
             if (a.mode_f == 0) ss_forward_wave<NPL, false, HYB, ALLLDS, true, H32>(a, ss_lds, c, lane);
             else if (a.mode_f == 1) ss_forward_wave<NPL, true, HYB, ALLLDS, true, H32>(a, ss_lds, c, lane);
@@ -1352,6 +1429,15 @@
         else ss_forward_light<NPL, ALLLDS, H32>(a, ss_lds, c, lane);
     } else {
         if (idle_b) return;
+        if (LIVE) {
+            if (a.mode_b == 0) {
+                if (a.halo) ss_backward_wave<NPL, false, HYB, ALLLDS, true, H32, true, 2>(a, ss_lds, c, lane);
+                else ss_backward_wave<NPL, false, HYB, ALLLDS, true, H32, true, 0>(a, ss_lds, c, lane);
+            } else if (a.mode_b == 1) {
+                if (a.full_b) ss_backward_wave<NPL, true, HYB, ALLLDS, true, H32, true, 1>(a, ss_lds, c, lane);
+                else ss_backward_wave<NPL, true, HYB, ALLLDS, true, H32, true, 0>(a, ss_lds, c, lane);
+            } else ss_backward_light<NPL, ALLLDS, H32, true>(a, ss_lds, c, lane);
+        } else
         if (NPL == 1 && !HYB && a.mixed) {
             if (a.mode_b == 0) ss_backward_wave<NPL, false, HYB, ALLLDS, true, H32>(a, ss_lds, c, lane);
             else if (a.mode_b == 1) ss_backward_wave<NPL, true, HYB, ALLLDS, true, H32>(a, ss_lds, c, lane);
diff --git a/smcpp_amd/csrc/engine_plans.hpp b/smcpp_amd/csrc/engine_plans.hpp
--- a/smcpp_amd/csrc/engine_plans.hpp
+++ b/smcpp_amd/csrc/engine_plans.hpp
@@ -464,15 +464,19 @@
     return true;
 }
 
-template <int NPL_, bool HYB_, bool ALL_, bool H32_ = false>
+template <int NPL_, bool HYB_, bool ALL_, bool H32_ = false, bool LIVE_ = false>
 static void launch_chain_ss_tt(const SsArgs &a, int ntasks, size_t shm, hipStream_t s, int wgw) {
-    lds_limit_once<k_chain_ss<NPL_, HYB_, ALL_, H32_>>();
-    hipLaunchKernelGGL((k_chain_ss<NPL_, HYB_, ALL_, H32_>), dim3(ntasks / wgw), dim3(64 * wgw), shm, s, a);
+    lds_limit_once<k_chain_ss<NPL_, HYB_, ALL_, LIVE_, H32_>>();
+    hipLaunchKernelGGL((k_chain_ss<NPL_, HYB_, ALL_, LIVE_, H32_>), dim3(ntasks / wgw), dim3(64 * wgw), shm, s, a);
+}
+static bool ss_all_lanes_live(int npl, const SsArgs &a) {
+    return npl == 1 && a.hyb_th == 0x7fffffff && a.mixed && a.M == 64 && a.Mp == 64 && a.K <= a.nlds;
 }
 template <int NPL_, bool HYB_>
 static void launch_chain_ss_t(const SsArgs &a, int ntasks, size_t shm, hipStream_t s, int wgw) {
     const bool h32_off = opt().off(smcpp_opt::O_SS_H32);
-    if (NPL_ == 1 && !HYB_ && a.K <= a.nlds && a.Mp <= 32 && !h32_off) launch_chain_ss_tt<NPL_, HYB_, true, NPL_ == 1 && !HYB_>(a, ntasks, shm, s, wgw);
+    if (NPL_ == 1 && !HYB_ && ss_all_lanes_live(NPL_, a)) launch_chain_ss_tt<NPL_, HYB_, true, false, NPL_ == 1 && !HYB_>(a, ntasks, shm, s, wgw);
+    else if (NPL_ == 1 && !HYB_ && a.K <= a.nlds && a.Mp <= 32 && !h32_off) launch_chain_ss_tt<NPL_, HYB_, true, NPL_ == 1 && !HYB_>(a, ntasks, shm, s, wgw);
     else if (a.K <= a.nlds) launch_chain_ss_tt<NPL_, HYB_, true>(a, ntasks, shm, s, wgw);
     else launch_chain_ss_tt<NPL_, HYB_, false>(a, ntasks, shm, s, wgw);
 }
diff --git a/smcpp_amd/csrc/engine_rccl.hpp b/smcpp_amd/csrc/engine_rccl.hpp
--- a/smcpp_amd/csrc/engine_rccl.hpp
+++ b/smcpp_amd/csrc/engine_rccl.hpp
@@ -194,19 +194,20 @@
     std::string s = "{";
     s += smcpp_opt::describe_options();
     if (im) {
-        char t[1024];
+        char t[1536];
         const int fam = im->ss_static ? (im->ss_hybrid ? 6 : 5) : im->chain_mode;
         snprintf(t, sizeof t,
                  ", \"plan\": {\"chain_family\": %d, \"scan_chains\": %s, \"hybrid_rows\": %s, \"states\": %d, \"states_padded\": %d, "
                  "\"states_per_lane\": %d, \"keys\": %d, \"eigen_keys\": %d, \"rows\": %lld, \"positions\": %lld, \"max_span\": %d, "
                  "\"chunks_forward\": %zu, \"chunks_backward\": %zu, \"wavefronts_per_simd\": %d, \"halo_pass\": %s, "
-                 "\"light_passes_forward\": %d, \"light_passes_backward\": %d, \"float_scans_in_stored_passes\": %s, "
+                 "\"light_passes_forward\": %d, \"light_passes_backward\": %d, \"float_scans_in_stored_passes\": %s, \"all_lanes_live\": %s, "
                  "\"passes_to_certificate\": %d, \"passes_launched\": %d, \"certificate_pass_launched_up_front\": %s, "
                  "\"save_gamma\": %s, \"eigen_free_statistics\": %s, \"per_row_gamma\": \"%s\", \"long_rows_cut\": %s, \"warm_start\": %s, \"host_threads\": %d}",
                  fam, im->ss_static ? "true" : "false", im->ss_hybrid ? "true" : "false", im->M, im->Mp, im->NPL, im->K, im->Ke,
                  (long long)(im->total_rows - im->n_contigs), (long long)im->ss_positions, im->ss_max_span, im->chunks.size(),
                  im->chunks_b.size(), im->ss_wpc, (im->ss_static && im->ss_args.halo) ? "true" : "false", im->ss_light_f, im->ss_light_b,
-                 (im->ss_static && im->ss_args.mixed) ? "true" : "false", im->last_ss_passes, im->ss_launched,
+                 (im->ss_static && im->ss_args.mixed) ? "true" : "false",
+                 (im->ss_static && ss_all_lanes_live(im->NPL, im->ss_args)) ? "true" : "false", im->last_ss_passes, im->ss_launched,
                  (opt().on(smcpp_opt::O_SS_CERT_PASS) || im->ss_need_cert_pass) ? "true" : "false", im->save_gamma ? "true" : "false",
                  im->eigfree ? "true" : "false", !im->save_gamma ? "none" : im->eigfree ? "scan steps" : im->stats_plan.gamma_form == StatsPlan::GAMMA_PIECES ? "eigen-power pieces + scan steps" : "eigensystem", im->split_spans ? "true" : "false",
                  im->warm_start ? "true" : "false", omp_get_max_threads());
diff --git a/smcpp_amd/csrc/kernels.hpp b/smcpp_amd/csrc/kernels.hpp
--- a/smcpp_amd/csrc/kernels.hpp
+++ b/smcpp_amd/csrc/kernels.hpp
@@ -1107,6 +1107,7 @@
                     acc[i][j] = __builtin_amdgcn_mfma_f64_16x16x4f64(xa[i], yb[j], acc[i][j], 0, 0, 0);
         }
     }
+    const double *red0 = nullptr;
     if (TEAM) {
         __shared__ double red[2][64 * 64];
         if (wv >= 2) {
@@ -1137,13 +1138,9 @@
         }
         __syncthreads();
         if (wv != 0) return;
-#pragma unroll
-        for (int i = 0; i < 4; ++i)
-#pragma unroll
-            for (int j = 0; j < 4; ++j)
-#pragma unroll
-                for (int rg = 0; rg < 4; ++rg) acc[i][j][rg] += red[0][((i * 4 + j) * 4 + rg) * 64 + lane];
-    }
+        red0 = red[0];
+    }
+    auto fin = [&](int i, int j, int rg) { return TEAM ? acc[i][j][rg] + red0[((i * 4 + j) * 4 + rg) * 64 + lane] : acc[i][j][rg]; };
     double *out = a.part + (size_t)blockIdx.x * Mp * Mp;
     if (MODE != 1) {
         const int col = kb + 4 * m;
@@ -1153,7 +1150,7 @@
             for (int rg = 0; rg < 4; ++rg) {
                 const int row = jb + 4 * (qd + 4 * rg) + i;
                 if (row < Mp && col < Mp)
-                    *reinterpret_cast<double4 *>(out + (size_t)row * Mp + col) = make_double4(acc[i][0][rg], acc[i][1][rg], acc[i][2][rg], acc[i][3][rg]);
+                    *reinterpret_cast<double4 *>(out + (size_t)row * Mp + col) = make_double4(fin(i, 0, rg), fin(i, 1, rg), fin(i, 2, rg), fin(i, 3, rg));
             }
         return;
     }
@@ -1165,7 +1162,7 @@
             for (int rg = 0; rg < 4; ++rg) {
                 const int row = jb + 16 * i + qd + 4 * rg;
                 const int col = kb + 16 * j + m;
-                if (row < Mp && col < Mp) out[(size_t)row * Mp + col] = acc[i][j][rg];
+                if (row < Mp && col < Mp) out[(size_t)row * Mp + col] = fin(i, j, rg);
             }
 }
 
```
